# lbcb-sci/raven

Measured on NVIDIA H100. Metric: overlaps/s, higher is better.
Workload: dtype u64

## Files before the change

### profiles/index_build_split.py

```python
from __future__ import annotations

import argparse
import ctypes as C
import json
import os
import subprocess
import sys

ROOT = os.path.dirname(os.path.dirname(os.path.abspath(__file__)))
sys.path.insert(0, ROOT)

SEED = 20260924
K, W, FREQ, KMAX = 15, 5, 0.001, 32
READS, GENOME, MEAN_LEN = 200_000, 50_000_000, 10_000

KERNELS = ("TierCountKernel", "TierScatterKernel", "RadixHistogramKernel", "RadixScanBinsKernel",
           "OnesweepPass", "PartitionPass", "GroupCountKernel", "BareCountKernel",
           "IndexTableKernel", "FillLongGaps")


def card():
    try:
        out = subprocess.run(["nvidia-smi", "--query-gpu=name,power.limit,clocks.max.sm",
                              "--format=csv,noheader"], capture_output=True, text=True,
                             timeout=30).stdout.strip().splitlines()
        return out[0] if out else "unknown"
    except (OSError, subprocess.SubprocessError):
        return "unknown"


def index_sizes(eng):
    v, o, n, nk = (C.POINTER(C.c_uint64)(), C.POINTER(C.c_uint64)(), C.c_uint64(0),
                   C.c_uint64(0))
    eng._check(eng.lib.rvn_index_records(eng.h, C.byref(v), C.byref(o), C.byref(n), C.byref(nk)))
    n_a = n.value
    vmax = max(v[n_a - 1], 1) if n_a else 1
    return n_a, int(eng.stats()["index_records"]), int(vmax).bit_length()


def algorithmic_bytes(name, n, n_a, n_b, passes_a):
    if "TierCountKernel" in name:
        return 4 * n
    if "TierScatterKernel" in name:
        return 4 * n + 8 * n_a + 12 * n_a + 4 * n_b
    if "RadixHistogramKernel<unsigned int>" in name:
        return 4 * (n_a + n_b)
    if "OnesweepPass<unsigned int, unsigned long" in name:
        return passes_a * 24 * n_a
    if "OnesweepPass<unsigned int, unsigned int, false>" in name:
        return 2 * 8 * n_b
    if "PartitionPass" in name:
        return 8 * n_b
    if "GroupCountKernel" in name or "BareCountKernel" in name:
        return 4 * n_b
    if "IndexTableKernel<unsigned int, true>" in name:
        return 4 * n_a
    return None


def main():
    ap = argparse.ArgumentParser()
    ap.add_argument("--steps", type=int, default=3)
    ap.add_argument("--warmup", type=int, default=2)
    ap.add_argument("--bare-count", default="0,1,8,16")
    ap.add_argument("--out", default=None, metavar="DIR",
                    help="also write the tables as DIR/index_build_split.json")
    a = ap.parse_args()

    import torch
    from torch.profiler import ProfilerActivity, profile

    if not torch.cuda.is_available():
        raise SystemExit("index_build_split.py needs a CUDA device")
    from bench import synth
    from raven_b200 import engine

    rs = synth.make_reads(SEED, GENOME, READS, MEAN_LEN)
    stream = torch.cuda.current_stream()
    eng = engine.Engine(device=0, stream=stream.cuda_stream)
    eng.configure(K, W)
    eng.upload(rs)

    def step():
        eng.find_overlaps_and_create_piles(FREQ, KMAX, False, 0, fetch=False)

    dev = card()
    print(f"card: {dev}")
    report = {"card": dev, "settings": {}}
    for setting in a.bare_count.split(","):
        if setting != "default":
            eng.set_option("bare_count", int(setting))
        for _ in range(a.warmup):
            step()
        torch.cuda.synchronize()
        eng.set_option("reset_stats", 1)
        with profile(activities=[ProfilerActivity.CUDA]) as prof:
            for _ in range(a.steps):
                step()
            torch.cuda.synchronize()
        phases = eng.timings()
        free, total = torch.cuda.mem_get_info()
        n_a, n, bits_a = index_sizes(eng)
        n_b = n - n_a
        passes_a = -(-bits_a // 10)
        per = {}
        for e in prof.events():
            if e.device_type != torch.autograd.DeviceType.CUDA:
                continue
            if not any(k in e.name for k in KERNELS):
                continue
            d = per.setdefault(e.name, [0.0, 0])
            d[0] += (e.time_range.end - e.time_range.start) / 1e3
            d[1] += 1
        rows = []
        for name, (ms, cnt) in sorted(per.items(), key=lambda x: -x[1][0]):
            ms_step, launches = ms / a.steps, cnt / a.steps
            b = algorithmic_bytes(name, n, n_a, n_b, passes_a)
            rate = (b / (ms_step * 1e-3) / 1e12) if b and ms_step > 0 else None
            short = name.replace("(anonymous namespace)::", "").replace("void ", "")
            short = short.replace("unsigned ", "u").replace("rvn::", "").split("(")[0]
            rows.append({"kernel": short, "ms_per_step": round(ms_step, 3),
                         "launches_per_step": launches,
                         "gbytes": None if b is None else round(b / 1e9, 3),
                         "tb_per_s": None if rate is None else round(rate, 3)})
        print(f"\nbare_count={setting}: {a.steps} steps, n={n} n_a={n_a} n_b={n_b} "
              f"(tier A: {bits_a} bits, {passes_a} passes); device memory in use after the "
              f"steps {(total - free) / 2**30:.2f} GiB")
        print(f"  phases (last step, ms): index_sort {phases.get('index_sort', 0):.2f}  "
              f"index_table {phases.get('index_table', 0):.2f}")
        print(f"  {'kernel':<58} {'ms/step':>8} {'launch':>6} {'GB':>7} {'TB/s':>6}")
        for r in rows:
            print(f"  {r['kernel'][:58]:<58} {r['ms_per_step']:8.3f} {r['launches_per_step']:6.1f} "
                  f"{'' if r['gbytes'] is None else r['gbytes']:>7} "
                  f"{'' if r['tb_per_s'] is None else r['tb_per_s']:>6}")
        report["settings"][setting] = {
            "n": n, "n_a": n_a, "n_b": n_b, "phases_ms": phases, "kernels": rows,
            "device_mem_used_gib": round((total - free) / 2**30, 3)}
    if a.out:
        os.makedirs(a.out, exist_ok=True)
        with open(os.path.join(a.out, "index_build_split.json"), "w") as f:
            json.dump(report, f, indent=1)
    eng.close()


if __name__ == "__main__":
    main()
```

### raven_b200/csrc/engine.cuh

```cuda
#pragma once

#include <string>
#include <vector>

#include "../../include/raven_b200.h"
#include "common.cuh"

namespace rvn {

struct Params {
  uint32_t k = 15, w = 5, bandwidth = 500, chain = 4, matches = 100;
  uint32_t gap = 10000;
};

constexpr uint32_t kSketchTile = 2048;
constexpr uint32_t kSketchThreads = 256;
constexpr uint32_t kMaxWindow = 256;

struct PhaseTimer {
  std::vector<const char*> names;
  std::vector<float> ms;
  std::vector<std::pair<cudaEvent_t, cudaEvent_t>> pending;
  std::vector<cudaEvent_t> pool;
};

struct Ctx {
  int device = 0;
  int sms = 132;
  cudaStream_t stream = nullptr;
  bool own_stream = false;
  int64_t async_upload = 0;
  cudaStream_t copy_stream = nullptr;
  cudaEvent_t up_fence = nullptr;
  std::vector<cudaEvent_t> up_events;
  std::vector<uint32_t> up_read_end;
  uint32_t up_chunks = 0;
  bool up_pending = false;
  bool p_off_uploaded = false;
  std::string err;
  Params prm;
  bool keep_hits = false;
  rvn_stats stats{};

  uint32_t n_reads = 0;
  uint64_t n_words = 0;
  DevBuf<uint64_t> d_words, d_woff;
  DevBuf<uint32_t> d_len, d_ids;
  std::vector<uint64_t> h_woff;
  std::vector<uint32_t> h_len, h_ids;
  bool ids_identity = true;
  uint32_t res_first = 0, res_last = 0;
  std::vector<uint64_t> h_tile_off;
  DevBuf<uint64_t> d_tile_off;
  DevBuf<uint32_t> d_tile_read;
  uint32_t tiles_k = 0;

  bool s_valid = false;
  uint32_t s_first = 0, s_last = 0;
  uint64_t s_n = 0;
  DevBuf<uint64_t> s_val, s_org, s_off;
  bool s_is32 = false;
  std::vector<uint64_t> h_s_off;
  DevBuf<uint32_t> tile_cnt;
  DevBuf<uint64_t> tile_out, tile_status;

  bool q_valid = false;
  uint32_t q_first = 0, q_last = 0;
  uint64_t q_n = 0;
  DevBuf<uint64_t> q_val, q_org, q_off;
  bool q_is32 = false;
  std::vector<uint64_t> h_q_off;
  bool qt_valid = false;
  uint32_t qt_first = 0, qt_last = 0;
  DevBuf<uint64_t> qt_val;
  DevBuf<uint32_t> qt_pos;
  int t_b_low = 0;
  uint64_t group_count_min = 0;
  bool i_from_sketch = false;
  int64_t self_join = 1;
  int64_t bare_count = 1;

  bool i_valid = false;
  uint32_t i_first = 0, i_last = 0;
  uint64_t i_n = 0, i_keys = 0;
  DevBuf<uint64_t> i_val, i_org, i_val_alt, i_org_alt;
  bool i_is32 = false;
  int i_shift = 0;
  uint64_t i_limit = ~0ULL;
  DevBuf<uint32_t> t_cnt;
  DevBuf<uint64_t> t_off, t_aval, t_aorg, t_b0, t_b1, t_b2, t_narrow;
  const uint32_t* t_sorted_b = nullptr;
  uint64_t t_nb = 0;
  bool t_b_sorted = true;
  DevBuf<uint32_t> t_bstart;
  int bare_cluster = 0;
  int bare_clusters = 0;
  uint64_t tier_min_records = 1ULL << 18;
  DevBuf<uint32_t> i_bucket;
  int i_bucket_bits = 0;
  DevBuf<uint64_t> i_gaps;
  DevBuf<uint64_t> i_hist;
  uint32_t occurrence = 0xFFFFFFFFu;
  bool i_sorted_ids = false;
  bool ids_ascending = true;
  DevBuf<uint8_t> sort_tmp;

  DevBuf<uint32_t> m_cnt, m_first;
  DevBuf<uint8_t> m_filt;
  DevBuf<uint64_t> m_hit_off;
  DevBuf<uint64_t> m_sq_key, m_sq_key2;
  DevBuf<uint32_t> m_sq_idx, m_sq_idx2;
  DevBuf<uint64_t> h_grp, h_pos;
  DevBuf<uint64_t> m_read_hit_off;
  uint64_t i_gen = 0, j_gen = 0;
  uint32_t j_occurrence = 0, j_first = 0;
  std::vector<uint64_t> h_j_off;
  DevBuf<uint64_t> j_off, j_packed;
  DevBuf<uint32_t> j_cursor;
  DevBuf<uint64_t> m_scratch64;
  DevBuf<uint32_t> m_scratch32, m_fallback;
  DevBuf<uint32_t> m_desc, m_desc_cnt, m_desc_idx, m_desc_cnt2, m_desc_idx2, m_gdiag,
      m_oidx, m_oidx2;
  DevBuf<uint64_t> m_gpos, m_group_loc, m_okey, m_okey2, m_starts;
  DevBuf<uint32_t> m_bounds;
  DevBuf<rvn_overlap> m_ovl_raw, m_ovl, m_ovl_tmp;
  DevBuf<uint64_t> m_ovl_loc;
  DevBuf<uint64_t> m_ovl_off;
  DevBuf<uint64_t> m_counter;
  DevBuf<uint32_t> m_filtered;
  DevBuf<uint64_t> m_filt_off;
  DevBuf<uint64_t> scan_tmp;
  uint64_t m_hits = 0;
  uint32_t m_first_read = 0, m_last_read = 0;

  PinBuf<rvn_overlap> r_ovl;
  PinBuf<uint64_t> r_ovl_off;
  PinBuf<uint32_t> r_filtered;
  PinBuf<uint64_t> r_filt_off;
  uint64_t r_n_ovl = 0;
  bool r_valid = false;
  PinBuf<uint64_t> r_hit_grp, r_hit_pos, r_hit_off;
  uint64_t r_n_hits = 0;

  PinBuf<uint64_t> x_val, x_org, x_off;

  DevBuf<int32_t> p_diff;
  DevBuf<uint16_t> p_data;
  DevBuf<uint64_t> p_off;
  DevBuf<rvn_overlap> p_ovl;

  int g_cur = 0;
  uint64_t g_total = 0;
  DevBuf<rvn_overlap> g_list[2], g_stage;
  DevBuf<uint64_t> g_off, g_off_alt, g_rhs_off, g_t_off, g_pairs;
  DevBuf<uint32_t> g_cnt, g_kept, g_key, g_idx, g_key2, g_idx2, g_rhs_cnt,
      g_total_cnt;

  DevBuf<uint32_t> po_win_first, po_seq_begin, po_seq_end, po_cons_len, po_cov, po_list;
  DevBuf<uint64_t> po_seq_off, po_d_cons_off;
  DevBuf<uint8_t> po_bases, po_quals, po_cons, po_status, po_scratch;
  std::vector<uint64_t> po_cons_off, po_out_off;
  std::vector<uint8_t> po_h_status, po_h_cons, po_out_cons;
  std::vector<uint32_t> po_h_clen, po_h_cov, po_out_cov;
  uint64_t po_cells = 0;
  uint32_t po_n_windows = 0;
  bool po_has_cov = false, poa_valid = false;

  PinBuf<rvn_overlap> st_ovl;
  PinBuf<uint64_t> st_ovl_off;
  PinBuf<uint16_t> st_pile;
  std::vector<uint64_t> st_pile_off;
  uint64_t st_mapped = 0;
  bool st_valid = false;
  bool st_piles_on_device = false;

  uint32_t own_mod = 1, own_rem = 0;

  DevBuf<uint64_t> ds_split_val, ds_split_org, ds_qsplit_val, ds_qsplit_org;
  DevBuf<uint64_t> ds_grouped_grp, ds_grouped_pos, ds_rel_off, ds_seg_start, ds_seg_base,
      ds_bounds, ds_q_off;
  DevBuf<uint32_t> ds_masked, ds_hit_lhs, ds_read_cnt, ds_flag, ds_own_ids;
  DevBuf<rvn_overlap> ds_ovl_split, ds_merged;
  PinBuf<rvn_overlap> ds_r_ovl;
  PinBuf<uint64_t> ds_r_ovl_off, ds_r_pile_off;
  PinBuf<uint16_t> ds_r_pile;
  uint32_t ds_n_own = 0;
  bool ds_results_valid = false;
  void* x_arena = nullptr;
  uint64_t x_cap = 0;
  uint32_t x_rank = 0;
  std::vector<void*> x_peers;
  std::vector<cudaStream_t> x_streams;

  PinBuf<uint64_t> pin64;

  PhaseTimer timer;
  uint64_t launches = 0;
};

void ExclusiveScanU32(Ctx& c, const uint32_t* in, uint64_t* out, uint64_t n);
uint64_t ReadU64(Ctx& c, const uint64_t* dptr);

void TimerBegin(Ctx& c, const char* name);
void TimerEnd(Ctx& c);
void TimerCollect(Ctx& c);
void TimerReset(Ctx& c);

void EnsureTiles(Ctx& c);
void EnsureSketch(Ctx& c, uint32_t first, uint32_t last);
void WaitUpload(Ctx& c);
void EnsureMicromizers(Ctx& c, uint32_t first, uint32_t last);
void EnsureThresholds(Ctx& c, uint32_t first, uint32_t last);

void BuildIndex(Ctx& c, uint32_t first, uint32_t last, bool minhash,
                uint64_t value_limit = ~0ULL);
uint64_t MaxMicromizerValue(Ctx& c, uint32_t first, uint32_t last);
void BuildIndexFrom(Ctx& c, ValView src_val, const uint64_t* src_org, uint64_t n,
                    uint64_t index_bases, uint64_t value_limit = ~0ULL, bool count_bare = false);

int RadixSortPairs(Ctx& c, const uint32_t* src_keys, uint32_t* keys_a, uint32_t* keys_b,
                   const uint64_t* src_vals, uint64_t* vals_a, uint64_t* vals_b, uint64_t n,
                   int begin_bit, int end_bit, bool descending = false);
int RadixSortPairs(Ctx& c, const uint64_t* src_keys, uint64_t* keys_a, uint64_t* keys_b,
                   const uint64_t* src_vals, uint64_t* vals_a, uint64_t* vals_b, uint64_t n,
                   int begin_bit, int end_bit, bool descending = false);
int RadixSortPairs(Ctx& c, const uint32_t* src_keys, uint32_t* keys_a, uint32_t* keys_b,
                   const uint32_t* src_vals, uint32_t* vals_a, uint32_t* vals_b, uint64_t n,
                   int begin_bit, int end_bit, bool descending = false);
int RadixSortPairs(Ctx& c, const uint64_t* src_keys, uint64_t* keys_a, uint64_t* keys_b,
                   const uint32_t* src_vals, uint32_t* vals_a, uint32_t* vals_b, uint64_t n,
                   int begin_bit, int end_bit, bool descending = false);
int RadixSortKeys(Ctx& c, const uint32_t* src_keys, uint32_t* keys_a, uint32_t* keys_b,
                  uint64_t n, int begin_bit, int end_bit);
void RadixPartitionKeys(Ctx& c, const uint32_t* src, uint32_t* dst, uint64_t n, int begin_bit,
                        int end_bit, uint32_t* bin_start);
uint64_t* IndexHistogram(Ctx& c);
uint32_t ThresholdFromHistogram(Ctx& c, const uint64_t* h_hist, uint64_t n_keys,
                                double frequency, bool* needs_long_runs);
uint32_t FilterIndex(Ctx& c, double frequency);

void MapRange(Ctx& c, uint32_t first, uint32_t last, bool avoid_equal,
              bool avoid_symmetric, bool minhash, bool want_filtered,
              bool fetch = true);

uint64_t ChainGroupedHits(Ctx& c, const uint64_t* hg, const uint64_t* hp,
                          const uint64_t* read_hit_off,
                          const std::vector<uint64_t>& h_rho, const uint32_t* lhs_ids,
                          uint32_t nr, uint64_t n_hits, uint64_t n_q);

void GatherReset(Ctx& c);
void GatherFlush(Ctx& c, const rvn_overlap* ovl, const uint64_t* q_ovl_off,
                 uint64_t m, uint32_t k0, uint32_t k1, uint64_t kmax);
void GatherFetch(Ctx& c);

void DistSketchSplit(Ctx& c, uint32_t first, uint32_t last, int which, uint32_t parts,
                     const uint64_t** d_val, const uint64_t** d_org, uint64_t* counts);
void DistHitsSplit(Ctx& c, const uint64_t* d_qval, const uint64_t* d_qorg, uint64_t n_q,
                   bool avoid_equal, bool avoid_symmetric, uint32_t parts, uint32_t n_query,
                   const uint64_t** d_grp, const uint64_t** d_pos, const uint32_t** d_lhs,
                   uint64_t* counts);
void DistChainOwned(Ctx& c, const uint64_t* d_grp, const uint64_t* d_pos,
                    const uint32_t* d_lhs, uint64_t n_hits, uint32_t n_seg,
                    const uint64_t* h_seg_off, uint32_t mod, uint32_t rem, uint32_t n_query,
                    const rvn_overlap** d_ovl, uint64_t* n_ovl);
void DistOverlapsSplit(Ctx& c, uint32_t parts, uint32_t self, const rvn_overlap** d_out,
                       uint64_t* counts);
void DistStage1Begin(Ctx& c, uint32_t parts, uint32_t rank);
void DistStage1Add(Ctx& c, const rvn_overlap* d_ovl, uint64_t n_ovl, uint32_t n_seg,
                   const uint64_t* h_seg_off, uint32_t n_query, uint64_t kmax, uint64_t qb);
void DistStage1End(Ctx& c);
void ArenaClosePeers(Ctx& c);
void ArenaExport(Ctx& c, uint64_t bytes, void* handle64);
void ArenaImport(Ctx& c, uint32_t parts, uint32_t rank, const void* handles);
void ArenaPut(Ctx& c, uint32_t dest, uint64_t dst_off, const void* d_src, uint64_t bytes);
void ArenaFlush(Ctx& c);
void ArenaRelease(Ctx& c);

void StagePileRegions(Ctx& c, uint32_t coverage, uint32_t* h_begin, uint32_t* h_end,
                      uint16_t* h_median, uint8_t* h_invalid);
void AlignBreakingPoints(Ctx& c, uint64_t n, const uint32_t* q_read, const uint32_t* q_begin,
                         const uint32_t* q_len, const uint8_t* strand, const uint32_t* t_read,
                         const uint32_t* t_begin, const uint32_t* t_len, uint32_t window,
                         const uint64_t* bp_off, int32_t* distance, uint32_t* bp);
void EditDistanceBatch(Ctx& c, uint64_t n, const uint32_t* lhs_read, const uint32_t* lhs_begin,
                       const uint32_t* lhs_len, const uint32_t* rhs_read,
                       const uint32_t* rhs_begin, const uint32_t* rhs_len,
                       const uint8_t* strand, const int32_t* limit, int32_t* out);

void PileAddLayersDevice(Ctx& c, uint16_t* d_data, const uint64_t* d_off,
                         const uint64_t* h_off, uint32_t n_piles,
                         const rvn_overlap* d_ovl, uint64_t n_ovl);

void PoaBatch(Ctx& c, uint32_t n_windows, const uint32_t* h_win_first,
              const uint64_t* h_seq_off, const uint8_t* h_bases, const uint8_t* h_quals,
              const uint32_t* h_seq_begin, const uint32_t* h_seq_end, int m, int n,
              int gap, bool trim, bool tgs, bool want_coverage);

void KmerComplexity(Ctx& c, const uint32_t* h_read_idx, const uint32_t* h_pos,
                    uint64_t n, uint32_t k, uint8_t* h_keep);

}
```

### raven_b200/csrc/index.cu

```cuda
#include <algorithm>
#include <cmath>

#include <cooperative_groups.h>

#include "engine.cuh"

namespace rvn {

namespace {

constexpr int kThreads = 256;

constexpr uint32_t kHistBins = 1u << 16;
constexpr uint32_t kSmemBins = 1024;

constexpr uint32_t kShortGap = 1024;
constexpr uint32_t kMaxLongGaps = 1u << 20;

template <typename ValT, bool kFill>
__global__ void __launch_bounds__(kThreads)
IndexTableKernel(const ValT* __restrict__ val, uint64_t n, int shift,
                 uint32_t n_buckets, uint32_t* __restrict__ bucket,
                 unsigned long long* __restrict__ hist, uint64_t* __restrict__ gaps) {
  __shared__ uint32_t sh[kSmemBins];
  __shared__ uint32_t keys;
  __shared__ uint32_t warp_first[kThreads / 32];
  for (uint32_t i = threadIdx.x; i < kSmemBins; i += kThreads) sh[i] = 0;
  if (threadIdx.x == 0) keys = 0;
  __syncthreads();
  const uint64_t stride = static_cast<uint64_t>(gridDim.x) * kThreads;
  for (uint64_t base = static_cast<uint64_t>(blockIdx.x) * kThreads; base <= n; base += stride) {
  const uint64_t i = base + threadIdx.x;
  bool start = false;
  uint32_t len = 0;
  uint64_t fill_lo = 0, mine = 0;
  uint32_t fill_cnt = 0;
  if (i <= n) {
    const uint64_t prev = i == 0 ? 0 : val[i - 1];
    const uint64_t cur = i == n ? 0 : val[i];
    const uint64_t lo = i == 0 ? 0 : (prev >> shift) + 1;
    const uint64_t hi = i == n ? n_buckets : (cur >> shift);
    if (kFill && hi >= lo) {
      if (hi + 1 - lo <= kShortGap) {
        fill_lo = lo;
        fill_cnt = static_cast<uint32_t>(hi + 1 - lo);
      } else {
        const unsigned long long g = atomicAdd(&hist[kHistBins + 1], 1ULL);
        if (g < kMaxLongGaps) {
          gaps[3 * g] = lo;
          gaps[3 * g + 1] = hi;
          gaps[3 * g + 2] = i;
        } else {
          for (uint64_t b = lo; b <= hi; ++b) bucket[b] = static_cast<uint32_t>(i);
        }
      }
    }
    start = i < n && (i == 0 || cur != prev);
    mine = cur;
  }
  {
    const uint32_t lane = threadIdx.x & 31, wid = threadIdx.x >> 5;
    const uint32_t marks = __ballot_sync(0xFFFFFFFFu, start || i == n);
    if (lane == 0) warp_first[wid] = marks ? static_cast<uint32_t>(__ffs(marks) - 1) : 32u;
    __syncthreads();
    if (start) {
      const uint32_t above = lane == 31 ? 0u : (marks & ~((2u << lane) - 1u));
      if (above) {
        len = static_cast<uint32_t>(__ffs(above) - 1) - lane;
      } else {
        len = 32 - lane;
        uint32_t w2 = wid + 1;
        while (w2 < kThreads / 32 && warp_first[w2] == 32u) {
          len += 32;
          ++w2;
        }
        if (w2 < kThreads / 32) {
          len += warp_first[w2];
        } else {
          uint64_t pos = base + kThreads;
          while (len < kHistBins - 1 && pos < n && val[pos] == mine) {
            ++pos;
            ++len;
          }
        }
      }
      if (len > kHistBins - 1) len = kHistBins - 1;
    }
    __syncthreads();
  }
  {
    const uint32_t lane = threadIdx.x & 31;
    uint32_t incl = fill_cnt;
#pragma unroll
    for (int d = 1; d < 32; d <<= 1) {
      const uint32_t o = __shfl_up_sync(0xFFFFFFFFu, incl, d);
      if (lane >= static_cast<uint32_t>(d)) incl += o;
    }
    const uint32_t rel = incl - fill_cnt;
    const uint32_t total = __shfl_sync(0xFFFFFFFFu, incl, 31);
    for (uint32_t t0 = 0; t0 < total; t0 += 32) {
      const uint32_t t = t0 + lane;
      uint32_t q = 0;
#pragma unroll
      for (uint32_t step = 16; step > 0; step >>= 1) {
        const uint32_t r = __shfl_sync(0xFFFFFFFFu, rel, q + step);
        if (r <= t) q += step;
      }
      const uint32_t qrel = __shfl_sync(0xFFFFFFFFu, rel, q);
      const uint64_t qlo = __shfl_sync(0xFFFFFFFFu, fill_lo, q);
      if (kFill && t < total) bucket[qlo + (t - qrel)] = static_cast<uint32_t>(base + (threadIdx.x & ~31u) + q);
    }
  }
  const uint32_t starts = __ballot_sync(0xFFFFFFFFu, start);
  if (start) {
    const uint32_t same = __match_any_sync(starts, len);
    if ((threadIdx.x & 31) == static_cast<uint32_t>(__ffs(same) - 1)) {
      if (len < kSmemBins) {
        atomicAdd(&sh[len], static_cast<uint32_t>(__popc(same)));
      } else {
        atomicAdd(&hist[len], static_cast<unsigned long long>(__popc(same)));
      }
    }
  }
  if ((threadIdx.x & 31) == 0 && starts) atomicAdd(&keys, static_cast<uint32_t>(__popc(starts)));

  }
  __syncthreads();
  for (uint32_t b = threadIdx.x; b < kSmemBins; b += kThreads) {
    if (sh[b]) atomicAdd(&hist[b], static_cast<unsigned long long>(sh[b]));
  }
  if (threadIdx.x == 0 && keys) atomicAdd(&hist[kHistBins], static_cast<unsigned long long>(keys));
}

__global__ void __launch_bounds__(kThreads)
FillLongGaps(const uint64_t* __restrict__ gaps, uint32_t* __restrict__ bucket) {
  const uint64_t lo = gaps[3ULL * blockIdx.x], hi = gaps[3ULL * blockIdx.x + 1];
  const uint32_t v = static_cast<uint32_t>(gaps[3ULL * blockIdx.x + 2]);
  for (uint64_t b = lo + threadIdx.x; b <= hi; b += kThreads) bucket[b] = v;
}

template <typename ValT>
__global__ void CollectLongRuns(const ValT* __restrict__ val, uint64_t n,
                                unsigned long long* __restrict__ counter,
                                uint32_t* __restrict__ out) {
  const uint64_t i = static_cast<uint64_t>(blockIdx.x) * blockDim.x + threadIdx.x;
  if (i >= n || (i > 0 && val[i] == val[i - 1])) return;
  if (i + (kHistBins - 2) >= n || val[i + (kHistBins - 2)] != val[i]) return;
  uint64_t len = kHistBins - 1;
  while (i + len < n && val[i + len] == val[i]) ++len;
  out[atomicAdd(counter, 1ULL)] = static_cast<uint32_t>(len);
}

__global__ void NarrowValuesKernel(const uint64_t* __restrict__ in, uint64_t n,
                                   uint32_t* __restrict__ out) {
  const uint64_t i = static_cast<uint64_t>(blockIdx.x) * blockDim.x + threadIdx.x;
  if (i < n) out[i] = static_cast<uint32_t>(in[i]);
}

constexpr uint32_t kTierTile = 4096;

__global__ void __launch_bounds__(kThreads)
TierCountKernel(const uint32_t* __restrict__ val, uint64_t n, uint32_t limit,
                uint32_t* __restrict__ tile_cnt) {
  __shared__ uint32_t sm[34];
  const uint64_t base = static_cast<uint64_t>(blockIdx.x) * kTierTile;
  uint32_t mine = 0;
#pragma unroll
  for (uint32_t i = 0; i < kTierTile / kThreads; ++i) {
    const uint64_t idx = base + i * kThreads + threadIdx.x;
    mine += (idx < n && val[idx] <= limit) ? 1u : 0u;
  }
  uint32_t total;
  BlockExclusiveSum<uint32_t, kThreads>(mine, sm, &total);
  if (threadIdx.x == 0) tile_cnt[blockIdx.x] = total;
}

__global__ void __launch_bounds__(kThreads, 4)
TierScatterKernel(const uint32_t* __restrict__ val, const uint64_t* __restrict__ org, uint64_t n,
                  uint32_t limit, const uint64_t* __restrict__ tile_off_a,
                  uint32_t* __restrict__ a_val, uint64_t* __restrict__ a_org,
                  uint32_t* __restrict__ b_val) {
  __shared__ uint32_t warp_a[kThreads / 32];
  const uint32_t lane = threadIdx.x & 31, warp = threadIdx.x >> 5;
  constexpr uint32_t kWarpSpan = kTierTile / (kThreads / 32);
  const uint64_t tile_base = static_cast<uint64_t>(blockIdx.x) * kTierTile;
  const uint64_t warp_base = tile_base + warp * kWarpSpan;
  uint32_t v[kWarpSpan / 32];
  uint32_t cnt = 0;
#pragma unroll
  for (uint32_t i = 0; i < kWarpSpan / 32; ++i) {
    const uint64_t idx = warp_base + i * 32 + lane;
    v[i] = idx < n ? val[idx] : 0xFFFFFFFFu;
  }
#pragma unroll
  for (uint32_t i = 0; i < kWarpSpan / 32; ++i) {
    const uint64_t idx = warp_base + i * 32 + lane;
    cnt += __popc(__ballot_sync(0xFFFFFFFFu, idx < n && v[i] <= limit));
  }
  if (lane == 0) warp_a[warp] = cnt;
  __syncthreads();
  uint64_t a_at = tile_off_a[blockIdx.x];
  for (uint32_t w = 0; w < warp; ++w) a_at += warp_a[w];
  uint64_t b_at = warp_base - a_at;
#pragma unroll
  for (uint32_t h = 0; h < kWarpSpan / 32; h += 8) {
    uint64_t o[8];
#pragma unroll
    for (uint32_t u = 0; u < 8; ++u) {
      const uint64_t idx = warp_base + (h + u) * 32 + lane;
      o[u] = (idx < n && v[h + u] <= limit) ? org[idx] : 0;
    }
#pragma unroll
    for (uint32_t u = 0; u < 8; ++u) {
      const uint32_t i = h + u;
      const uint64_t idx = warp_base + i * 32 + lane;
      const bool in = idx < n;
      const bool is_a = in && v[i] <= limit;
      const uint32_t ma = __ballot_sync(0xFFFFFFFFu, is_a);
      const uint32_t mb = __ballot_sync(0xFFFFFFFFu, in && !is_a);
      const uint32_t below = (1u << lane) - 1u;
      if (is_a) {
        const uint64_t d = a_at + __popc(ma & below);
        a_val[d] = v[i];
        a_org[d] = o[u];
      } else if (in) {
        b_val[b_at + __popc(mb & below)] = v[i];
      }
      a_at += __popc(ma);
      b_at += __popc(mb);
    }
  }
}

__global__ void MaxU64Kernel(const uint64_t* __restrict__ v, uint64_t n,
                             unsigned long long* __restrict__ out) {
  unsigned long long m = 0;
  const uint64_t stride = static_cast<uint64_t>(gridDim.x) * blockDim.x;
  for (uint64_t i = static_cast<uint64_t>(blockIdx.x) * blockDim.x + threadIdx.x; i < n;
       i += stride) {
    m = max(m, static_cast<unsigned long long>(v[i]));
  }
#pragma unroll
  for (int d = 16; d > 0; d >>= 1) m = max(m, __shfl_xor_sync(0xFFFFFFFFu, m, d));
  if ((threadIdx.x & 31) == 0) atomicMax(out, m);
}

constexpr uint32_t kGroupChunk = 4096;
constexpr int kGroupLowBits = 10;

__global__ void __launch_bounds__(kThreads)
GroupCountKernel(const uint32_t* __restrict__ key, uint64_t n, unsigned long long* __restrict__ hist) {
  __shared__ uint32_t sh[kSmemBins];
  __shared__ __align__(16) uint32_t cnt[kThreads / 32][1u << kGroupLowBits];
  __shared__ uint32_t keys_total;
  for (uint32_t i = threadIdx.x; i < kSmemBins; i += kThreads) sh[i] = 0;
  if (threadIdx.x == 0) keys_total = 0;
  __syncthreads();
  const uint32_t lane = threadIdx.x & 31, wid = threadIdx.x >> 5;
  uint32_t* my = cnt[wid];
  const uint32_t low_mask = (1u << kGroupLowBits) - 1;
  uint32_t h1 = 0, h2 = 0, h3 = 0, h4 = 0, nkeys = 0;
  const uint64_t n_chunks = (n + kGroupChunk - 1) / kGroupChunk;
  for (uint64_t chunk = static_cast<uint64_t>(blockIdx.x) * (kThreads / 32) + wid; chunk < n_chunks;
       chunk += static_cast<uint64_t>(gridDim.x) * (kThreads / 32)) {
    const uint64_t start = chunk * kGroupChunk;
    const uint64_t end = min(n, start + kGroupChunk);
    uint64_t pos = start;
    if (start > 0) {
      const uint32_t gprev = key[start - 1] >> kGroupLowBits;
      while (true) {
        const uint64_t idx = pos + lane;
        const bool in = idx < n && (key[idx] >> kGroupLowBits) == gprev;
        const uint32_t m = __ballot_sync(0xFFFFFFFFu, in);
        const uint32_t c = m == 0xFFFFFFFFu ? 32u : static_cast<uint32_t>(__ffs(~m) - 1);
        pos += c;
        if (c < 32) break;
      }
    }
    while (pos < end) {
      const uint32_t g = key[pos] >> kGroupLowBits;
      uint4* my4 = reinterpret_cast<uint4*>(my);
#pragma unroll
      for (uint32_t t = 0; t < (1u << kGroupLowBits) / 128; ++t) my4[t * 32 + lane] = make_uint4(0, 0, 0, 0);
      __syncwarp();
      bool open = true;
      while (open) {
        uint32_t k4[4];
#pragma unroll
        for (uint32_t u = 0; u < 4; ++u) {
          const uint64_t idx = pos + u * 32 + lane;
          k4[u] = idx < n ? key[idx] : ~(g << kGroupLowBits);
        }
#pragma unroll
        for (uint32_t u = 0; u < 4; ++u) {
          if (open) {
            const bool in = (k4[u] >> kGroupLowBits) == g;
            const uint32_t m = __ballot_sync(0xFFFFFFFFu, in);
            if (in) atomicAdd(&my[k4[u] & low_mask], 1u);
            const uint32_t c = m == 0xFFFFFFFFu ? 32u : static_cast<uint32_t>(__ffs(~m) - 1);
            pos += c;
            open = c == 32;
          }
        }
      }
      __syncwarp();
#pragma unroll
      for (uint32_t t = 0; t < (1u << kGroupLowBits) / 128; ++t) {
        const uint4 q = my4[t * 32 + lane];
        if ((q.x | q.y | q.z | q.w) == 0) continue;
        const uint32_t cs[4] = {q.x, q.y, q.z, q.w};
#pragma unroll
        for (int x = 0; x < 4; ++x) {
          const uint32_t c = cs[x];
          if (c == 0) continue;
          ++nkeys;
          if (c <= 4) {
            h1 += c == 1;
            h2 += c == 2;
            h3 += c == 3;
            h4 += c == 4;
          } else if (c < kSmemBins) {
            atomicAdd(&sh[c], 1u);
          } else {
            atomicAdd(&hist[min(c, kHistBins - 1)], 1ULL);
          }
        }
      }
      __syncwarp();
    }
  }
#pragma unroll
  for (int d = 16; d > 0; d >>= 1) {
    h1 += __shfl_xor_sync(0xFFFFFFFFu, h1, d);
    h2 += __shfl_xor_sync(0xFFFFFFFFu, h2, d);
    h3 += __shfl_xor_sync(0xFFFFFFFFu, h3, d);
    h4 += __shfl_xor_sync(0xFFFFFFFFu, h4, d);
    nkeys += __shfl_xor_sync(0xFFFFFFFFu, nkeys, d);
  }
  if (lane == 0) {
    atomicAdd(&sh[1], h1);
    atomicAdd(&sh[2], h2);
    atomicAdd(&sh[3], h3);
    atomicAdd(&sh[4], h4);
    atomicAdd(&keys_total, nkeys);
  }
  __syncthreads();
  for (uint32_t i = threadIdx.x; i < kSmemBins; i += kThreads) {
    if (sh[i]) atomicAdd(&hist[i], static_cast<unsigned long long>(sh[i]));
  }
  if (threadIdx.x == 0 && keys_total) {
    atomicAdd(&hist[kHistBins], static_cast<unsigned long long>(keys_total));
  }
}

constexpr int kBareBucketBits = 10;
constexpr int kBareThreads = 1024;
constexpr int kBareSlotBits = 15;

__global__ void __launch_bounds__(kBareThreads, 1)
BareCountKernel(const uint32_t* __restrict__ key, uint64_t n, const uint32_t* __restrict__ bstart,
                uint32_t first_bucket, uint32_t n_buckets, int span_bits, int slot_bits,
                unsigned long long* __restrict__ hist) {
  extern __shared__ __align__(16) uint32_t bare_smem[];
  __shared__ uint32_t keys_total;
  namespace cg = cooperative_groups;
  cg::cluster_group cluster = cg::this_cluster();
  const uint32_t csize = cluster.num_blocks();
  const uint32_t crank = cluster.block_rank();
  const uint32_t n_slots = 1u << slot_bits;
  uint32_t* ctr = bare_smem;
  uint32_t* sh = bare_smem + n_slots;
  for (uint32_t i = threadIdx.x; i < n_slots; i += kBareThreads) ctr[i] = 0;
  for (uint32_t i = threadIdx.x; i < kSmemBins; i += kBareThreads) sh[i] = 0;
  if (threadIdx.x == 0) keys_total = 0;
  const uint32_t ctr_addr = static_cast<uint32_t>(__cvta_generic_to_shared(ctr));
  const uint32_t span_mask = (1u << span_bits) - 1u;
  const uint32_t sweep_span = n_slots * csize;
  const uint32_t slot_mask = n_slots - 1u;
  uint32_t h1 = 0, h2 = 0, h3 = 0, h4 = 0, nkeys = 0;
  cluster.sync();
  const uint32_t n_clusters = gridDim.x / csize;
  for (uint32_t b = first_bucket + blockIdx.x / csize; b < n_buckets; b += n_clusters) {
    const uint64_t lo = bstart ? bstart[b] : 0;
    const uint64_t hi = bstart && b + 1 < n_buckets ? bstart[b + 1] : n;
    if (lo >= hi) continue;
    for (uint64_t s0 = 0; s0 <= span_mask; s0 += sweep_span) {
      constexpr int kUnroll = 4;
      const uint64_t stride = static_cast<uint64_t>(csize) * kBareThreads;
      for (uint64_t i0 = lo + crank * kBareThreads + threadIdx.x; i0 < hi; i0 += kUnroll * stride) {
        uint32_t k4[kUnroll];
#pragma unroll
        for (int u = 0; u < kUnroll; ++u) {
          const uint64_t i = i0 + u * stride;
          k4[u] = i < hi ? key[i] : 0u;
        }
#pragma unroll
        for (int u = 0; u < kUnroll; ++u) {
          const uint64_t v = static_cast<uint64_t>(k4[u] & span_mask) - s0;
          if (i0 + u * stride < hi && v < sweep_span) {
            const uint32_t owner = static_cast<uint32_t>(v) >> slot_bits;
            const uint32_t local = ctr_addr + 4u * (static_cast<uint32_t>(v) & slot_mask);
            uint32_t remote;
            asm volatile("mapa.shared::cluster.u32 %0, %1, %2;" : "=r"(remote) : "r"(local), "r"(owner));
            asm volatile("red.relaxed.cluster.shared::cluster.add.u32 [%0], 1;" ::"r"(remote) : "memory");
          }
        }
      }
      cluster.sync();
      for (uint32_t t = threadIdx.x; t < n_slots; t += kBareThreads) {
        const uint32_t c = ctr[t];
        if (c == 0) continue;
        ctr[t] = 0;
        ++nkeys;
        if (c <= 4) {
          h1 += c == 1;
          h2 += c == 2;
          h3 += c == 3;
          h4 += c == 4;
        } else if (c < kSmemBins) {
          atomicAdd(&sh[c], 1u);
        } else {
          atomicAdd(&hist[min(c, kHistBins - 1)], 1ULL);
        }
      }
      cluster.sync();
    }
  }
#pragma unroll
  for (int d = 16; d > 0; d >>= 1) {
    h1 += __shfl_xor_sync(0xFFFFFFFFu, h1, d);
    h2 += __shfl_xor_sync(0xFFFFFFFFu, h2, d);
    h3 += __shfl_xor_sync(0xFFFFFFFFu, h3, d);
    h4 += __shfl_xor_sync(0xFFFFFFFFu, h4, d);
    nkeys += __shfl_xor_sync(0xFFFFFFFFu, nkeys, d);
  }
  if ((threadIdx.x & 31) == 0) {
    atomicAdd(&sh[1], h1);
    atomicAdd(&sh[2], h2);
    atomicAdd(&sh[3], h3);
    atomicAdd(&sh[4], h4);
    atomicAdd(&keys_total, nkeys);
  }
  __syncthreads();
  for (uint32_t i = threadIdx.x; i < kSmemBins; i += kBareThreads) {
    if (sh[i]) atomicAdd(&hist[i], static_cast<unsigned long long>(sh[i]));
  }
  if (threadIdx.x == 0 && keys_total) {
    atomicAdd(&hist[kHistBins], static_cast<unsigned long long>(keys_total));
  }
}

void BareCount(Ctx& c, const uint32_t* keys, uint64_t n, int key_bits, uint32_t limit,
               const uint32_t* bstart, unsigned long long* hist) {
  const int span_bits = bstart ? key_bits - kBareBucketBits : key_bits;
  const uint32_t n_buckets = bstart ? (1u << kBareBucketBits) : 1u;
  const uint32_t first_bucket = bstart ? (limit >> span_bits) : 0u;
  if (c.bare_cluster == 0) {
    const int size = c.bare_count > 1 ? static_cast<int>(c.bare_count) : 8;
    const size_t smem = ((1u << kBareSlotBits) + kSmemBins) * sizeof(uint32_t);
    RVN_CUDA(cudaFuncSetAttribute(BareCountKernel, cudaFuncAttributeMaxDynamicSharedMemorySize,
                                  static_cast<int>(smem)));
    RVN_CUDA(cudaFuncSetAttribute(BareCountKernel, cudaFuncAttributeNonPortableClusterSizeAllowed, 1));
    cudaLaunchConfig_t cfg = {};
    cfg.gridDim = dim3(static_cast<unsigned>(size));
    cfg.blockDim = dim3(kBareThreads);
    cfg.dynamicSmemBytes = smem;
    cudaLaunchAttribute attr[1];
    attr[0].id = cudaLaunchAttributeClusterDimension;
    attr[0].val.clusterDim.x = static_cast<unsigned>(size);
    attr[0].val.clusterDim.y = 1;
    attr[0].val.clusterDim.z = 1;
    cfg.attrs = attr;
    cfg.numAttrs = 1;
    int clusters = 0;
    RVN_CUDA(cudaOccupancyMaxActiveClusters(&clusters, BareCountKernel, &cfg));
    if (clusters < 1) throw CudaError("BareCountKernel: a cluster does not fit the device");
    c.bare_cluster = size;
    c.bare_clusters = clusters;
  }
  const int csize = c.bare_cluster;
  int log_c = 0;
  while ((1 << log_c) < csize) ++log_c;
  const int slot_bits = std::max(0, std::min(kBareSlotBits, span_bits - log_c));
  const unsigned clusters =
      static_cast<unsigned>(std::min<uint64_t>(n_buckets - first_bucket, c.bare_clusters));
  cudaLaunchConfig_t cfg = {};
  cfg.gridDim = dim3(clusters * csize);
  cfg.blockDim = dim3(kBareThreads);
  cfg.dynamicSmemBytes = ((1u << slot_bits) + kSmemBins) * sizeof(uint32_t);
  cfg.stream = c.stream;
  cudaLaunchAttribute attr[1];
  attr[0].id = cudaLaunchAttributeClusterDimension;
  attr[0].val.clusterDim.x = static_cast<unsigned>(csize);
  attr[0].val.clusterDim.y = 1;
  attr[0].val.clusterDim.z = 1;
  cfg.attrs = attr;
  cfg.numAttrs = 1;
  RVN_CUDA(cudaLaunchKernelEx(&cfg, BareCountKernel, keys, n, bstart, first_bucket, n_buckets,
                              span_bits, slot_bits, hist));
  RVN_LAUNCH_CHECK();
  ++c.launches;
}

}

uint64_t MaxMicromizerValue(Ctx& c, uint32_t first, uint32_t last) {
  EnsureThresholds(c, first, last);
  if (last <= first) return 0;
  if (!c.s_is32) return ~0ULL;
  uint64_t* w = c.m_counter.reserve(8);
  RVN_CUDA(cudaMemsetAsync(w, 0, sizeof(uint64_t), c.stream));
  const uint64_t n = last - first;
  MaxU64Kernel<<<std::min<unsigned>(CeilDiv(n, 256), c.sms * 8), 256, 0, c.stream>>>(
      c.qt_val.get(), n, reinterpret_cast<unsigned long long*>(w));
  RVN_LAUNCH_CHECK();
  ++c.launches;
  return ReadU64(c, w);
}

void BuildIndex(Ctx& c, uint32_t first, uint32_t last, bool minhash, uint64_t value_limit) {
  c.i_valid = false;
  c.occurrence = 0xFFFFFFFFu;
  EnsureSketch(c, first, last);
  ValView src_val{c.s_val.get(), c.s_is32 ? 1 : 0};
  const uint64_t* src_org = c.s_org.get();
  uint64_t n = c.s_n;
  if (minhash) {
    EnsureMicromizers(c, first, last);
    src_val = ValView{c.q_val.get(), c.q_is32 ? 1 : 0};
    src_org = c.q_org.get();
    n = c.q_n;
  }
  uint64_t bases = 0;
  for (uint32_t r = first; r < last; ++r) bases += c.h_len[r];
  c.i_first = first;
  c.i_last = last;
  BuildIndexFrom(c, src_val, src_org, n, bases, minhash ? ~0ULL : value_limit,
                 true);
  c.i_sorted_ids = c.ids_ascending;
  c.i_from_sketch = !minhash;
}

void BuildIndexFrom(Ctx& c, ValView src_val, const uint64_t* src_org, uint64_t n,
                    uint64_t index_bases, uint64_t value_limit, bool count_bare) {
  c.i_valid = false;
  c.i_sorted_ids = false;
  c.i_from_sketch = false;
  c.occurrence = 0xFFFFFFFFu;
  ++c.i_gen;
  if (n >= 0xFFFFFFFFULL) {
    throw LimitError("index batch holds 2^32 or more minimizers");
  }
  c.i_n = n;
  c.i_keys = 0;
  if (!src_val.is32 && 2 * c.prm.k <= 30 && n > 0) {
    uint32_t* narrow = reinterpret_cast<uint32_t*>(c.t_narrow.reserve(n / 2 + 2));
    NarrowValuesKernel<<<CeilDiv(n, kThreads), kThreads, 0, c.stream>>>(
        static_cast<const uint64_t*>(src_val.p), n, narrow);
    RVN_LAUNCH_CHECK();
    ++c.launches;
    src_val = ValView{narrow, 1};
  }
  const bool is32 = src_val.is32 != 0;
  c.i_is32 = is32;

  const int key_bits = static_cast<int>(2 * c.prm.k);
  const uint64_t value_mask = key_bits >= 64 ? ~0ULL : ((1ULL << key_bits) - 1);
  const bool tiered = is32 && value_limit < value_mask && n >= c.tier_min_records;
  const uint32_t limit32 = static_cast<uint32_t>(value_limit);
  c.i_limit = tiered ? value_limit : ~0ULL;
  uint64_t n_a = n, n_b = 0;
  const uint32_t* sorted_b = nullptr;
  const bool bare = tiered && count_bare && c.bare_count != 0;
  const uint32_t* bstart = nullptr;

  TimerBegin(c, "index_sort");
  if (tiered) {
    const uint32_t* src32 = static_cast<const uint32_t*>(src_val.p);
    const uint64_t tiles = (n + kTierTile - 1) / kTierTile;
    uint32_t* tcnt = c.t_cnt.reserve(tiles + 1);
    uint64_t* toff = c.t_off.reserve(tiles + 2);
    TierCountKernel<<<static_cast<unsigned>(tiles), kThreads, 0, c.stream>>>(src32, n, limit32,
                                                                          tcnt);
    ExclusiveScanU32(c, tcnt, toff, tiles);
    n_a = ReadU64(c, toff + tiles);
    n_b = n - n_a;
    uint32_t* a_val = reinterpret_cast<uint32_t*>(c.t_aval.reserve(n_a / 2 + 2));
    uint64_t* a_org = c.t_aorg.reserve(n_a + 1);
    uint32_t* b_src = reinterpret_cast<uint32_t*>(c.t_b0.reserve(n_b / 2 + 2));
    TierScatterKernel<<<static_cast<unsigned>(tiles), kThreads, 0, c.stream>>>(
        src32, src_org, n, limit32, toff, a_val, a_org, b_src);
    RVN_LAUNCH_CHECK();
    c.launches += 2;
    int bits_a = 1;
    while (bits_a < key_bits && (value_limit >> bits_a) != 0) ++bits_a;
    c.i_val.reserve(n_a / 2 + 2);
    c.i_val_alt.reserve(n_a / 2 + 2);
    c.i_org.reserve(n_a + 1);
    c.i_org_alt.reserve(n_a + 1);
    if (n_a > 0) {
      const int where = RadixSortPairs(c, a_val, reinterpret_cast<uint32_t*>(c.i_val.get()),
                                       reinterpret_cast<uint32_t*>(c.i_val_alt.get()), a_org,
                                       c.i_org.get(), c.i_org_alt.get(), n_a, 0, bits_a);
      if (where == 1) {
        c.i_val.swap(c.i_val_alt);
        c.i_org.swap(c.i_org_alt);
      }
    }
    uint32_t* b1 = reinterpret_cast<uint32_t*>(c.t_b1.reserve(n_b / 2 + 2));
    if (bare) {
      c.t_b2.release();
      c.t_b_low = 0;
      c.t_b_sorted = false;
      sorted_b = n_b > 0 ? b_src : nullptr;
      if (n_b > 0 && key_bits > 2 * kBareBucketBits) {
        uint32_t* starts = c.t_bstart.reserve(1u << kBareBucketBits);
        RadixPartitionKeys(c, b_src, b1, n_b, key_bits - kBareBucketBits, key_bits, starts);
        sorted_b = b1;
        bstart = starts;
      }
    } else {
      uint32_t* b2 = reinterpret_cast<uint32_t*>(c.t_b2.reserve(n_b / 2 + 2));
      const uint64_t n_groups = ((value_mask - value_limit) >> kGroupLowBits) + 1;
      c.t_b_low = (key_bits > 2 * kGroupLowBits && n_b / n_groups >= c.group_count_min)
                      ? kGroupLowBits
                      : 0;
      c.t_b_sorted = c.t_b_low == 0;
      if (n_b > 0) {
        const int where = RadixSortKeys(c, b_src, b1, b2, n_b, c.t_b_low, key_bits);
        sorted_b = where < 0 ? b_src : (where == 0 ? b1 : b2);
      }
    }
    c.t_sorted_b = sorted_b;
    c.t_nb = n_b;
  } else {
    const uint64_t val_elems = is32 ? n / 2 + 2 : n + 1;
    c.i_val.reserve(val_elems);
    c.i_val_alt.reserve(val_elems);
    c.i_org.reserve(n + 1);
    c.i_org_alt.reserve(n + 1);
    if (n > 0) {
      int where;
      if (is32) {
        where = RadixSortPairs(c, static_cast<const uint32_t*>(src_val.p),
                               reinterpret_cast<uint32_t*>(c.i_val.get()),
                               reinterpret_cast<uint32_t*>(c.i_val_alt.get()), src_org,
                               c.i_org.get(), c.i_org_alt.get(), n, 0, key_bits);
      } else {
        where = RadixSortPairs(c, static_cast<const uint64_t*>(src_val.p), c.i_val.get(),
                               c.i_val_alt.get(), src_org, c.i_org.get(), c.i_org_alt.get(), n, 0,
                               key_bits);
      }
      if (where == 1) {
        c.i_val.swap(c.i_val_alt);
        c.i_org.swap(c.i_org_alt);
      }
    }
    c.t_sorted_b = nullptr;
    c.t_nb = 0;
    c.t_b_sorted = true;
  }
  c.i_n = n_a;
  TimerEnd(c);
  const uint64_t* kv = c.i_val.get();

  TimerBegin(c, "index_table");
  int top_bits = key_bits;
  if (tiered) {
    top_bits = 1;
    while (top_bits < key_bits && (value_limit >> top_bits) != 0) ++top_bits;
  }
  int bits = 8;
  while (bits < 28 && (1ULL << (bits + 1)) <= n_a) ++bits;
  bits = std::min<int>(bits, top_bits);
  c.i_bucket_bits = bits;
  const int shift = top_bits - bits;
  c.i_shift = shift;
  const uint32_t n_buckets =
      tiered ? static_cast<uint32_t>((value_limit >> shift) + 1) : (1u << bits);
  uint32_t* bucket = c.i_bucket.reserve(n_buckets + 2ULL);
  static_assert(sizeof(unsigned long long) == sizeof(uint64_t), "");
  uint64_t* hist = c.i_hist.reserve(kHistBins + 8);
  RVN_CUDA(cudaMemsetAsync(hist, 0, (kHistBins + 8) * sizeof(uint64_t), c.stream));
  uint64_t* gaps = c.i_gaps.reserve(3ULL * kMaxLongGaps);
  const unsigned grid = std::min<unsigned>(CeilDiv(n_a + 1, kThreads), c.sms * 8);
  if (is32) {
    IndexTableKernel<uint32_t, true><<<grid, kThreads, 0, c.stream>>>(
        reinterpret_cast<const uint32_t*>(kv), n_a, shift, n_buckets, bucket,
        reinterpret_cast<unsigned long long*>(hist), gaps);
    if (tiered && n_b > 0) {
      if (bare) {
        BareCount(c, sorted_b, n_b, key_bits, limit32, bstart,
                  reinterpret_cast<unsigned long long*>(hist));
        --c.launches;
      } else if (c.t_b_low) {
        GroupCountKernel<<<std::min<unsigned>(CeilDiv(n_b, kGroupChunk * (kThreads / 32)), c.sms * 6),
                           kThreads, 0, c.stream>>>(sorted_b, n_b,
                                                    reinterpret_cast<unsigned long long*>(hist));
      } else {
        IndexTableKernel<uint32_t, false>
            <<<std::min<unsigned>(CeilDiv(n_b + 1, kThreads), c.sms * 8), kThreads, 0, c.stream>>>(
                sorted_b, n_b, 0, 0, nullptr, reinterpret_cast<unsigned long long*>(hist), nullptr);
      }
      ++c.launches;
    }
  } else {
    IndexTableKernel<uint64_t, true><<<grid, kThreads, 0, c.stream>>>(
        kv, n_a, shift, n_buckets, bucket, reinterpret_cast<unsigned long long*>(hist), gaps);
  }
  RVN_LAUNCH_CHECK();
  ++c.launches;
  uint64_t* hk = c.pin64.reserve(8);
  RVN_CUDA(cudaMemcpyAsync(hk, hist + kHistBins, 2 * sizeof(uint64_t), cudaMemcpyDeviceToHost,
                           c.stream));
  RVN_CUDA(cudaStreamSynchronize(c.stream));
  c.i_keys = hk[0];
  const uint64_t n_long = std::min<uint64_t>(hk[1], kMaxLongGaps);
  if (n_long) {
    FillLongGaps<<<static_cast<unsigned>(n_long), kThreads, 0, c.stream>>>(gaps, bucket);
    RVN_LAUNCH_CHECK();
    ++c.launches;
  }
  TimerEnd(c);

  c.stats.index_bases = index_bases;
  c.stats.index_records = n;
  c.stats.index_keys = c.i_keys;
  c.i_valid = true;
}

uint64_t* IndexHistogram(Ctx& c) {
  return c.i_hist.get();
}

uint32_t ThresholdFromHistogram(Ctx& c, const uint64_t* h, uint64_t n_keys,
                                double frequency, bool* needs_long_runs) {
  (void)c;
  *needs_long_runs = false;
  std::size_t rank = static_cast<std::size_t>((1 - frequency) * static_cast<double>(n_keys));
  if (rank >= n_keys) rank = n_keys - 1;
  uint64_t cum = 0;
  for (uint32_t len = 0; len + 1 < kHistBins; ++len) {
    cum += h[len];
    if (cum > rank) return len + 1;
  }
  *needs_long_runs = true;
  return 0;
}

uint32_t FilterIndex(Ctx& c, double frequency) {
  if (!(0 <= frequency && frequency <= 1)) {
    throw InvalidArgument(
        "[ram::MinimizerEngine::Filter] error: invalid frequency");
  }
  if (!c.i_valid) throw StateError("Filter before Minimize");
  if (frequency == 0 || c.i_keys == 0) {
    c.occurrence = 0xFFFFFFFFu;
    return c.occurrence;
  }
  uint64_t* hist = IndexHistogram(c);
  std::vector<uint64_t> h(kHistBins);
  RVN_CUDA(cudaMemcpyAsync(h.data(), hist, kHistBins * sizeof(uint64_t),
                           cudaMemcpyDeviceToHost, c.stream));
  RVN_CUDA(cudaStreamSynchronize(c.stream));
  bool long_runs = false;
  uint32_t occ = ThresholdFromHistogram(c, h.data(), c.i_keys, frequency, &long_runs);
  if (long_runs) {
    uint64_t cum = 0;
    for (uint32_t len = 0; len + 1 < kHistBins; ++len) cum += h[len];
    std::size_t rank = static_cast<std::size_t>((1 - frequency) * static_cast<double>(c.i_keys));
    if (rank >= c.i_keys) rank = c.i_keys - 1;
    const uint64_t n_long = h[kHistBins - 1];
    uint32_t* out = c.m_cnt.reserve(n_long + 1);
    uint64_t* counter = c.m_counter.reserve(8);
    RVN_CUDA(cudaMemsetAsync(counter, 0, sizeof(uint64_t), c.stream));
    if (c.i_is32) {
      CollectLongRuns<uint32_t><<<CeilDiv(c.i_n, kThreads), kThreads, 0, c.stream>>>(
          reinterpret_cast<const uint32_t*>(c.i_val.get()), c.i_n,
          reinterpret_cast<unsigned long long*>(counter), out);
      if (c.t_sorted_b && c.t_nb && !c.t_b_sorted) {
        uint32_t* bufs[3] = {reinterpret_cast<uint32_t*>(c.t_b0.get()),
                             reinterpret_cast<uint32_t*>(c.t_b1.get()),
                             reinterpret_cast<uint32_t*>(c.t_b2.get())};
        uint32_t* src = nullptr;
        for (uint32_t* p : bufs) {
          if (p == c.t_sorted_b) src = p;
        }
        uint32_t* other = src == bufs[0] ? bufs[1] : bufs[0];
        const int where = RadixSortKeys(c, src, other, src, c.t_nb, 0,
                                        static_cast<int>(2 * c.prm.k));
        c.t_sorted_b = where == 0 ? other : src;
        c.t_b_low = 0;
        c.t_b_sorted = true;
      }
      if (c.t_sorted_b && c.t_nb) {
        CollectLongRuns<uint32_t><<<CeilDiv(c.t_nb, kThreads), kThreads, 0, c.stream>>>(
            c.t_sorted_b, c.t_nb, reinterpret_cast<unsigned long long*>(counter), out);
      }
    } else {
      CollectLongRuns<uint64_t><<<CeilDiv(c.i_n, kThreads), kThreads, 0, c.stream>>>(
          c.i_val.get(), c.i_n, reinterpret_cast<unsigned long long*>(counter), out);
    }
    RVN_LAUNCH_CHECK();
    ++c.launches;
    std::vector<uint32_t> lens(n_long);
    RVN_CUDA(cudaMemcpyAsync(lens.data(), out, n_long * sizeof(uint32_t),
                             cudaMemcpyDeviceToHost, c.stream));
    RVN_CUDA(cudaStreamSynchronize(c.stream));
    std::sort(lens.begin(), lens.end());
    occ = lens[rank - cum] + 1;
  }
  c.occurrence = occ;
  c.stats.occurrence = c.occurrence;
  return c.occurrence;
}

}
```

### raven_b200/csrc/radix.cu

```cuda
#include <algorithm>

#include "engine.cuh"

namespace rvn {

namespace {

constexpr int kRadixMaxBits = 10;
constexpr int kBins = 1 << kRadixMaxBits;
constexpr int kThreads = 256;
constexpr int kWarps = kThreads / 32;
constexpr int kBinsPerThread = kBins / kThreads;
constexpr int kMaxPasses = 8;
template <typename KeyT>
struct Items {
  static constexpr int value = sizeof(KeyT) == 4 ? 32 : 16;
};

constexpr uint32_t kFlagAggregate = 1u << 30;
constexpr uint32_t kFlagPrefix = 2u << 30;
constexpr uint32_t kFlagMask = 3u << 30;
constexpr uint32_t kValueMask = ~kFlagMask;

struct PassPlan {
  int n_passes;
  int begin[kMaxPasses];
  int bits[kMaxPasses];
};

template <typename KeyT>
__device__ __forceinline__ uint32_t Digit(KeyT key, KeyT flip, int begin, uint32_t mask) {
  return static_cast<uint32_t>((key ^ flip) >> begin) & mask;
}

template <typename KeyT>
__global__ void __launch_bounds__(kThreads)
RadixHistogramKernel(const KeyT* __restrict__ keys, uint64_t n, PassPlan plan, KeyT flip,
                     unsigned long long* __restrict__ hist) {
  extern __shared__ uint32_t sh_hist[];
  const int total = plan.n_passes * kBins;
  for (int i = threadIdx.x; i < total; i += kThreads) sh_hist[i] = 0;
  __syncthreads();
  const uint64_t stride = static_cast<uint64_t>(gridDim.x) * kThreads;
  for (uint64_t i = static_cast<uint64_t>(blockIdx.x) * kThreads + threadIdx.x; i < n;
       i += stride) {
    const KeyT k = keys[i];
#pragma unroll
    for (int p = 0; p < kMaxPasses; ++p) {
      if (p < plan.n_passes) {
        atomicAdd(&sh_hist[p * kBins + Digit<KeyT>(k, flip, plan.begin[p],
                                                    (1u << plan.bits[p]) - 1u)], 1u);
      }
    }
  }
  __syncthreads();
  for (int i = threadIdx.x; i < total; i += kThreads) {
    if (sh_hist[i]) atomicAdd(&hist[i], static_cast<unsigned long long>(sh_hist[i]));
  }
}

__global__ void __launch_bounds__(kBins)
RadixScanBinsKernel(const unsigned long long* __restrict__ hist, int n_passes,
                    uint32_t* __restrict__ bin_base) {
  __shared__ uint32_t sm[34];
  for (int p = 0; p < n_passes; ++p) {
    const uint32_t v = static_cast<uint32_t>(hist[p * kBins + threadIdx.x]);
    uint32_t total;
    const uint32_t ex = BlockExclusiveSum<uint32_t, kBins>(v, sm, &total);
    bin_base[p * kBins + threadIdx.x] = ex;
  }
}

__device__ __forceinline__ void ChainTileCounts(uint32_t* __restrict__ status, uint32_t tile,
                                                const uint32_t (&cnt)[kBinsPerThread],
                                                uint32_t (&excl)[kBinsPerThread]) {
  uint4* st4 = reinterpret_cast<uint4*>(status);
  const uint64_t my4 = static_cast<uint64_t>(tile) * (kBins / 4) + threadIdx.x;
#pragma unroll
  for (int j = 0; j < kBinsPerThread; ++j) excl[j] = 0;
  static_assert(kBinsPerThread == 4, "one uint4 of status words per thread");
  if (tile > 0) {
    uint4 agg;
    agg.x = kFlagAggregate | cnt[0];
    agg.y = kFlagAggregate | cnt[1];
    agg.z = kFlagAggregate | cnt[2];
    agg.w = kFlagAggregate | cnt[3];
    asm volatile("st.volatile.global.v4.u32 [%0], {%1, %2, %3, %4};" ::"l"(st4 + my4),
                 "r"(agg.x), "r"(agg.y), "r"(agg.z), "r"(agg.w)
                 : "memory");
    constexpr int kLook = 4;
    uint32_t open = 0xF;
    int64_t p = static_cast<int64_t>(tile) - 1;
    while (open) {
      uint4 v[kLook];
#pragma unroll
      for (int u = 0; u < kLook; ++u) {
        const int64_t q = p - u;
        if (q >= 0) {
          const uint4* src = st4 + static_cast<uint64_t>(q) * (kBins / 4) + threadIdx.x;
          asm volatile("ld.volatile.global.v4.u32 {%0, %1, %2, %3}, [%4];"
                       : "=r"(v[u].x), "=r"(v[u].y), "=r"(v[u].z), "=r"(v[u].w)
                       : "l"(src)
                       : "memory");
        } else {
          v[u] = make_uint4(kFlagPrefix, kFlagPrefix, kFlagPrefix, kFlagPrefix);
        }
      }
      int used = 0;
#pragma unroll
      for (int u = 0; u < kLook; ++u) {
        const uint32_t vv[4] = {v[u].x, v[u].y, v[u].z, v[u].w};
        const bool ready = (vv[0] & kFlagMask) && (vv[1] & kFlagMask) && (vv[2] & kFlagMask) &&
                           (vv[3] & kFlagMask);
        if (used == u && ready && open) {
#pragma unroll
          for (int j = 0; j < kBinsPerThread; ++j) {
            if (open & (1u << j)) {
              excl[j] += vv[j] & kValueMask;
              if ((vv[j] & kFlagMask) == kFlagPrefix) open &= ~(1u << j);
            }
          }
          used = u + 1;
        }
      }
      p -= used;
    }
  }
  uint4 pre;
  pre.x = kFlagPrefix | (excl[0] + cnt[0]);
  pre.y = kFlagPrefix | (excl[1] + cnt[1]);
  pre.z = kFlagPrefix | (excl[2] + cnt[2]);
  pre.w = kFlagPrefix | (excl[3] + cnt[3]);
  asm volatile("st.volatile.global.v4.u32 [%0], {%1, %2, %3, %4};" ::"l"(st4 + my4), "r"(pre.x),
               "r"(pre.y), "r"(pre.z), "r"(pre.w)
               : "memory");
}

template <typename KeyT, typename ValT, bool HAS_VAL>
struct __align__(16) PassSmem {
  static constexpr int kTile = kThreads * Items<KeyT>::value;
  uint16_t warp_hist[kWarps][kBins];
  uint32_t bin_off[kBins];
  uint32_t bin_dst[kBins];
  uint32_t scan[34];
  uint32_t tile;
  uint16_t slot_digit[HAS_VAL ? kTile : 2];
  union {
    KeyT keys[kTile];
    ValT vals[HAS_VAL ? kTile : 1];
  } stage;
};

template <typename KeyT, typename ValT, bool HAS_VAL>
__global__ void __launch_bounds__(kThreads, 2)
OnesweepPass(const KeyT* __restrict__ keys_in, KeyT* __restrict__ keys_out,
             const ValT* __restrict__ vals_in, ValT* __restrict__ vals_out, uint32_t n,
             KeyT flip, int begin_bit, int pass_bits, const uint32_t* __restrict__ bin_base,
             uint32_t* __restrict__ bin_next, uint32_t* __restrict__ status,
             unsigned int* __restrict__ ticket) {
  extern __shared__ __align__(16) unsigned char smem_raw[];
  using Smem = PassSmem<KeyT, ValT, HAS_VAL>;
  constexpr int kItems = Items<KeyT>::value;
  constexpr int kTile = kThreads * kItems;
  constexpr int kWarpTile = 32 * kItems;
  Smem& sm = *reinterpret_cast<Smem*>(smem_raw);
  const uint32_t lane = threadIdx.x & 31, warp = threadIdx.x >> 5;
  const uint32_t lanemask_lt = (1u << lane) - 1u;
  const uint32_t dmask = (1u << pass_bits) - 1u;

  if (threadIdx.x == 0) sm.tile = atomicAdd(ticket, 1u);
  {
    uint32_t* w = reinterpret_cast<uint32_t*>(&sm.warp_hist[0][0]);
#pragma unroll
    for (int i = 0; i < kWarps * kBins / 2 / kThreads; ++i) w[i * kThreads + threadIdx.x] = 0;
  }
  __syncthreads();
  const uint32_t tile = sm.tile;
  const uint64_t tile_base = static_cast<uint64_t>(tile) * kTile;
  const uint32_t tile_count =
      static_cast<uint32_t>(min(static_cast<uint64_t>(kTile), static_cast<uint64_t>(n) - tile_base));

  KeyT key[kItems];
  const uint32_t warp_base = warp * kWarpTile;
#pragma unroll
  for (int i = 0; i < kItems; ++i) {
    const uint32_t t = warp_base + i * 32 + lane;
    key[i] = t < tile_count ? keys_in[tile_base + t] : static_cast<KeyT>(0);
  }

  constexpr int kHalf = kItems / 2;
  ValT early[HAS_VAL ? kHalf : 1];
  if (HAS_VAL) {
#pragma unroll
    for (int i = 0; i < kHalf; ++i) {
      const uint32_t t = warp_base + i * 32 + lane;
      early[i] = t < tile_count ? vals_in[tile_base + t] : ValT(0);
    }
  }

  uint16_t rank[kItems];
  uint16_t* my_hist = sm.warp_hist[warp];
#pragma unroll
  for (int i = 0; i < kItems; ++i) {
    const uint32_t t = warp_base + i * 32 + lane;
    const bool valid = t < tile_count;
    const uint32_t d = valid ? Digit<KeyT>(key[i], flip, begin_bit, dmask) : 0u;
    uint32_t peers = __ballot_sync(0xFFFFFFFFu, valid);
#pragma unroll
    for (int bit = 0; bit < kRadixMaxBits; ++bit) {
      const bool one = (d >> bit) & 1u;
      const uint32_t vote = __ballot_sync(0xFFFFFFFFu, one);
      peers &= one ? vote : ~vote;
    }
    if (!valid) peers = 1u << lane;
    const uint32_t leader = __ffs(peers) - 1;
    uint32_t before = 0;
    if (lane == leader && valid) {
      before = my_hist[d];
      my_hist[d] = static_cast<uint16_t>(before + __popc(peers));
    }
    before = __shfl_sync(0xFFFFFFFFu, before, leader);
    rank[i] = static_cast<uint16_t>(before + __popc(peers & lanemask_lt));
    __syncwarp();
  }
  __syncthreads();

  uint32_t cnt[kBinsPerThread];
  uint32_t mine = 0;
#pragma unroll
  for (int j = 0; j < kBinsPerThread; ++j) {
    const uint32_t b = threadIdx.x * kBinsPerThread + j;
    uint32_t c = 0;
#pragma unroll
    for (int w = 0; w < kWarps; ++w) {
      const uint32_t x = sm.warp_hist[w][b];
      sm.warp_hist[w][b] = static_cast<uint16_t>(c);
      c += x;
    }
    cnt[j] = c;
    mine += c;
  }
  uint32_t total;
  uint32_t ex = BlockExclusiveSum<uint32_t, kThreads>(mine, sm.scan, &total);
#pragma unroll
  for (int j = 0; j < kBinsPerThread; ++j) {
    sm.bin_off[threadIdx.x * kBinsPerThread + j] = ex;
    ex += cnt[j];
  }

  {
    uint32_t excl[kBinsPerThread];
    ChainTileCounts(status, tile, cnt, excl);
#pragma unroll
    for (int j = 0; j < kBinsPerThread; ++j) {
      const uint32_t b = threadIdx.x * kBinsPerThread + j;
      const uint32_t base = bin_base[b];
      sm.bin_dst[b] = base + excl[j] - sm.bin_off[b];
      if (tile == gridDim.x - 1) bin_next[b] = base + excl[j] + cnt[j];
    }
  }
  __syncthreads();

#pragma unroll
  for (int i = 0; i < kItems; ++i) {
    const uint32_t t = warp_base + i * 32 + lane;
    if (t < tile_count) {
      const uint32_t d = Digit<KeyT>(key[i], flip, begin_bit, dmask);
      const uint32_t slot = sm.bin_off[d] + sm.warp_hist[warp][d] + rank[i];
      rank[i] = static_cast<uint16_t>(slot);
      if (HAS_VAL) sm.slot_digit[slot] = static_cast<uint16_t>(d);
    }
  }

  if (HAS_VAL) {
    ValT late[kHalf];
#pragma unroll
    for (int i = 0; i < kHalf; ++i) {
      const uint32_t t = warp_base + (kHalf + i) * 32 + lane;
      late[i] = t < tile_count ? vals_in[tile_base + t] : ValT(0);
    }
#pragma unroll
    for (int i = 0; i < kHalf; ++i) {
      const uint32_t t = warp_base + i * 32 + lane;
      if (t < tile_count) sm.stage.vals[rank[i]] = early[i];
    }
#pragma unroll
    for (int i = 0; i < kHalf; ++i) {
      const uint32_t t = warp_base + (kHalf + i) * 32 + lane;
      if (t < tile_count) sm.stage.vals[rank[kHalf + i]] = late[i];
    }
    __syncthreads();
#pragma unroll
    for (int i = 0; i < kItems; ++i) {
      const uint32_t s = i * kThreads + threadIdx.x;
      if (s < tile_count) vals_out[sm.bin_dst[sm.slot_digit[s]] + s] = sm.stage.vals[s];
    }
    __syncthreads();
  }

#pragma unroll
  for (int i = 0; i < kItems; ++i) {
    const uint32_t t = warp_base + i * 32 + lane;
    if (t < tile_count) sm.stage.keys[rank[i]] = key[i];
  }
  __syncthreads();
#pragma unroll
  for (int i = 0; i < kItems; ++i) {
    const uint32_t s = i * kThreads + threadIdx.x;
    if (s < tile_count) {
      const KeyT k = sm.stage.keys[s];
      keys_out[sm.bin_dst[Digit<KeyT>(k, flip, begin_bit, dmask)] + s] = k;
    }
  }
}

struct PartitionSmem {
  uint32_t bin_cnt[kBins];
  uint32_t bin_off[kBins];
  uint32_t bin_dst[kBins];
  uint32_t scan[34];
  uint32_t tile;
  uint32_t keys[kThreads * Items<uint32_t>::value];
};

__global__ void __launch_bounds__(kThreads, 2)
PartitionPass(const uint32_t* __restrict__ keys_in, uint32_t* __restrict__ keys_out, uint32_t n,
              int begin_bit, int pass_bits, const uint32_t* __restrict__ bin_base,
              uint32_t* __restrict__ bin_next, uint32_t* __restrict__ status,
              unsigned int* __restrict__ ticket) {
  extern __shared__ __align__(16) unsigned char smem_raw[];
  PartitionSmem& sm = *reinterpret_cast<PartitionSmem*>(smem_raw);
  constexpr int kItems = Items<uint32_t>::value;
  constexpr int kTile = kThreads * kItems;
  constexpr int kWarpTile = 32 * kItems;
  const uint32_t lane = threadIdx.x & 31, warp = threadIdx.x >> 5;
  const uint32_t dmask = (1u << pass_bits) - 1u;

  if (threadIdx.x == 0) sm.tile = atomicAdd(ticket, 1u);
#pragma unroll
  for (int j = 0; j < kBinsPerThread; ++j) sm.bin_cnt[j * kThreads + threadIdx.x] = 0;
  __syncthreads();
  const uint32_t tile = sm.tile;
  const uint64_t tile_base = static_cast<uint64_t>(tile) * kTile;
  const uint32_t tile_count =
      static_cast<uint32_t>(min(static_cast<uint64_t>(kTile), static_cast<uint64_t>(n) - tile_base));

  uint32_t key[kItems];
  const uint32_t warp_base = warp * kWarpTile;
#pragma unroll
  for (int i = 0; i < kItems; ++i) {
    const uint32_t t = warp_base + i * 32 + lane;
    key[i] = t < tile_count ? keys_in[tile_base + t] : 0u;
  }
  uint16_t rank[kItems];
#pragma unroll
  for (int i = 0; i < kItems; ++i) {
    const uint32_t t = warp_base + i * 32 + lane;
    if (t < tile_count) {
      rank[i] = static_cast<uint16_t>(atomicAdd(&sm.bin_cnt[(key[i] >> begin_bit) & dmask], 1u));
    }
  }
  __syncthreads();

  uint32_t cnt[kBinsPerThread];
  uint32_t mine = 0;
#pragma unroll
  for (int j = 0; j < kBinsPerThread; ++j) {
    cnt[j] = sm.bin_cnt[threadIdx.x * kBinsPerThread + j];
    mine += cnt[j];
  }
  uint32_t total;
  uint32_t ex = BlockExclusiveSum<uint32_t, kThreads>(mine, sm.scan, &total);
#pragma unroll
  for (int j = 0; j < kBinsPerThread; ++j) {
    sm.bin_off[threadIdx.x * kBinsPerThread + j] = ex;
    ex += cnt[j];
  }
  {
    uint32_t excl[kBinsPerThread];
    ChainTileCounts(status, tile, cnt, excl);
#pragma unroll
    for (int j = 0; j < kBinsPerThread; ++j) {
      const uint32_t b = threadIdx.x * kBinsPerThread + j;
      const uint32_t base = bin_base[b];
      sm.bin_dst[b] = base + excl[j] - sm.bin_off[b];
      if (tile == gridDim.x - 1) bin_next[b] = base + excl[j] + cnt[j];
    }
  }
  __syncthreads();

#pragma unroll
  for (int i = 0; i < kItems; ++i) {
    const uint32_t t = warp_base + i * 32 + lane;
    if (t < tile_count) sm.keys[sm.bin_off[(key[i] >> begin_bit) & dmask] + rank[i]] = key[i];
  }
  __syncthreads();
#pragma unroll
  for (int i = 0; i < kItems; ++i) {
    const uint32_t s = i * kThreads + threadIdx.x;
    if (s < tile_count) {
      const uint32_t k = sm.keys[s];
      keys_out[sm.bin_dst[(k >> begin_bit) & dmask] + s] = k;
    }
  }
}

PassPlan MakePlan(int begin_bit, int end_bit) {
  PassPlan plan{};
  const int total = std::max(0, end_bit - begin_bit);
  const int np = (total + kRadixMaxBits - 1) / kRadixMaxBits;
  if (np > kMaxPasses) throw InvalidArgument("radix sort: too many key bits");
  plan.n_passes = np;
  int at = begin_bit;
  for (int p = 0; p < np; ++p) {
    const int b = (total - (at - begin_bit) + (np - p) - 1) / (np - p);
    plan.begin[p] = at;
    plan.bits[p] = b;
    at += b;
  }
  return plan;
}

template <typename KeyT, typename ValT, bool HAS_VAL>
int SortImpl(Ctx& c, const KeyT* src_keys, KeyT* keys_a, KeyT* keys_b, const ValT* src_vals,
             ValT* vals_a, ValT* vals_b, uint64_t n, int begin_bit, int end_bit,
             bool descending) {
  if (n >= 0xFFFFFFFFULL) throw LimitError("radix sort of 2^32 or more records");
  const PassPlan plan = MakePlan(begin_bit, end_bit);
  if (plan.n_passes == 0 || n == 0) return -1;
  using Smem = PassSmem<KeyT, ValT, HAS_VAL>;
  constexpr uint64_t kTile = Smem::kTile;
  const KeyT flip = descending ? static_cast<KeyT>(~static_cast<KeyT>(0)) : static_cast<KeyT>(0);
  const uint64_t portion = ((1ULL << 30) - 1) / kTile * kTile;
  const uint64_t n_portions = (n + portion - 1) / portion;
  const uint64_t max_tiles = (std::min(n, portion) + kTile - 1) / kTile;
  const size_t hist_bytes = sizeof(uint64_t) * plan.n_passes * kBins;
  const size_t base_bytes = sizeof(uint32_t) * plan.n_passes * kBins;
  const size_t ticket_bytes = sizeof(unsigned int) * kMaxPasses * 8;
  if (plan.n_passes * n_portions > kMaxPasses * 8) throw LimitError("radix sort: too many launches");
  const size_t status_bytes = sizeof(uint32_t) * max_tiles * kBins;
  const size_t head = hist_bytes + 2 * base_bytes + ticket_bytes;
  uint8_t* scratch = c.sort_tmp.reserve(head + status_bytes + 256);
  auto* hist = reinterpret_cast<unsigned long long*>(scratch);
  uint32_t* bases[2] = {reinterpret_cast<uint32_t*>(scratch + hist_bytes),
                        reinterpret_cast<uint32_t*>(scratch + hist_bytes + base_bytes)};
  auto* ticket = reinterpret_cast<unsigned int*>(scratch + hist_bytes + 2 * base_bytes);
  auto* status = reinterpret_cast<uint32_t*>(scratch + head);
  RVN_CUDA(cudaMemsetAsync(scratch, 0, head, c.stream));
  const unsigned hgrid =
      static_cast<unsigned>(std::min<uint64_t>((n + kThreads - 1) / kThreads, c.sms * 8));
  RadixHistogramKernel<KeyT><<<hgrid, kThreads, sizeof(uint32_t) * plan.n_passes * kBins,
                               c.stream>>>(src_keys, n, plan, flip, hist);
  RadixScanBinsKernel<<<1, kBins, 0, c.stream>>>(hist, plan.n_passes, bases[0]);
  RVN_LAUNCH_CHECK();
  c.launches += 2;

  auto kern = OnesweepPass<KeyT, ValT, HAS_VAL>;
  RVN_CUDA(cudaFuncSetAttribute(kern, cudaFuncAttributeMaxDynamicSharedMemorySize,
                                static_cast<int>(sizeof(Smem))));
  const KeyT* kin = src_keys;
  const ValT* vin = src_vals;
  int where = -1;
  unsigned launch = 0;
  for (int p = 0; p < plan.n_passes; ++p) {
    const int to = where == 0 ? 1 : 0;
    KeyT* kout = to == 0 ? keys_a : keys_b;
    ValT* vout = to == 0 ? vals_a : vals_b;
    int cur = 0;
    for (uint64_t q = 0; q < n_portions; ++q) {
      const uint64_t first = q * portion;
      const uint64_t cnt = std::min(portion, n - first);
      const uint64_t tiles = (cnt + kTile - 1) / kTile;
      RVN_CUDA(cudaMemsetAsync(status, 0, sizeof(uint32_t) * tiles * kBins, c.stream));
      kern<<<static_cast<unsigned>(tiles), kThreads, sizeof(Smem), c.stream>>>(
          kin + first, kout, HAS_VAL ? vin + first : vin, vout, static_cast<uint32_t>(cnt), flip,
          plan.begin[p], plan.bits[p], bases[cur] + p * kBins, bases[cur ^ 1] + p * kBins, status,
          ticket + launch);
      RVN_LAUNCH_CHECK();
      ++c.launches;
      ++launch;
      cur ^= 1;
    }
    kin = kout;
    vin = vout;
    where = to;
  }
  return where;
}

}

int RadixSortPairs(Ctx& c, const uint32_t* src_keys, uint32_t* keys_a, uint32_t* keys_b,
                   const uint64_t* src_vals, uint64_t* vals_a, uint64_t* vals_b, uint64_t n,
                   int begin_bit, int end_bit, bool descending) {
  return SortImpl<uint32_t, uint64_t, true>(c, src_keys, keys_a, keys_b, src_vals, vals_a, vals_b,
                                            n, begin_bit, end_bit, descending);
}
int RadixSortPairs(Ctx& c, const uint64_t* src_keys, uint64_t* keys_a, uint64_t* keys_b,
                   const uint64_t* src_vals, uint64_t* vals_a, uint64_t* vals_b, uint64_t n,
                   int begin_bit, int end_bit, bool descending) {
  return SortImpl<uint64_t, uint64_t, true>(c, src_keys, keys_a, keys_b, src_vals, vals_a, vals_b,
                                            n, begin_bit, end_bit, descending);
}
int RadixSortPairs(Ctx& c, const uint32_t* src_keys, uint32_t* keys_a, uint32_t* keys_b,
                   const uint32_t* src_vals, uint32_t* vals_a, uint32_t* vals_b, uint64_t n,
                   int begin_bit, int end_bit, bool descending) {
  return SortImpl<uint32_t, uint32_t, true>(c, src_keys, keys_a, keys_b, src_vals, vals_a, vals_b,
                                            n, begin_bit, end_bit, descending);
}
int RadixSortPairs(Ctx& c, const uint64_t* src_keys, uint64_t* keys_a, uint64_t* keys_b,
                   const uint32_t* src_vals, uint32_t* vals_a, uint32_t* vals_b, uint64_t n,
                   int begin_bit, int end_bit, bool descending) {
  return SortImpl<uint64_t, uint32_t, true>(c, src_keys, keys_a, keys_b, src_vals, vals_a, vals_b,
                                            n, begin_bit, end_bit, descending);
}
int RadixSortKeys(Ctx& c, const uint32_t* src_keys, uint32_t* keys_a, uint32_t* keys_b, uint64_t n,
                  int begin_bit, int end_bit) {
  return SortImpl<uint32_t, uint32_t, false>(c, src_keys, keys_a, keys_b, nullptr, nullptr, nullptr,
                                             n, begin_bit, end_bit, false);
}

void RadixPartitionKeys(Ctx& c, const uint32_t* src, uint32_t* dst, uint64_t n, int begin_bit,
                        int end_bit, uint32_t* bin_start) {
  if (n >= 0xFFFFFFFFULL) throw LimitError("radix partition of 2^32 or more records");
  if (end_bit - begin_bit < 1 || end_bit - begin_bit > kRadixMaxBits) {
    throw InvalidArgument("radix partition: 1 to 10 key bits");
  }
  PassPlan plan{};
  plan.n_passes = 1;
  plan.begin[0] = begin_bit;
  plan.bits[0] = end_bit - begin_bit;
  constexpr uint64_t kTile = kThreads * Items<uint32_t>::value;
  const uint64_t portion = ((1ULL << 30) - 1) / kTile * kTile;
  const uint64_t n_portions = (n + portion - 1) / portion;
  const uint64_t max_tiles = (std::min(n, portion) + kTile - 1) / kTile;
  const size_t hist_bytes = sizeof(uint64_t) * kBins;
  const size_t base_bytes = sizeof(uint32_t) * kBins;
  const size_t ticket_bytes = sizeof(unsigned int) * kMaxPasses * 8;
  if (n_portions > kMaxPasses * 8) throw LimitError("radix partition: too many launches");
  const size_t head = hist_bytes + 2 * base_bytes + ticket_bytes;
  const size_t status_bytes = sizeof(uint32_t) * max_tiles * kBins;
  uint8_t* scratch = c.sort_tmp.reserve(head + status_bytes + 256);
  auto* hist = reinterpret_cast<unsigned long long*>(scratch);
  uint32_t* bases[2] = {reinterpret_cast<uint32_t*>(scratch + hist_bytes),
                        reinterpret_cast<uint32_t*>(scratch + hist_bytes + base_bytes)};
  auto* ticket = reinterpret_cast<unsigned int*>(scratch + hist_bytes + 2 * base_bytes);
  auto* status = reinterpret_cast<uint32_t*>(scratch + head);
  RVN_CUDA(cudaMemsetAsync(scratch, 0, head, c.stream));
  if (n == 0) {
    RVN_CUDA(cudaMemsetAsync(bin_start, 0, base_bytes, c.stream));
    return;
  }
  const unsigned hgrid =
      static_cast<unsigned>(std::min<uint64_t>((n + kThreads - 1) / kThreads, c.sms * 8));
  RadixHistogramKernel<uint32_t><<<hgrid, kThreads, sizeof(uint32_t) * kBins, c.stream>>>(
      src, n, plan, 0u, hist);
  RadixScanBinsKernel<<<1, kBins, 0, c.stream>>>(hist, 1, bases[0]);
  RVN_LAUNCH_CHECK();
  c.launches += 2;
  RVN_CUDA(cudaMemcpyAsync(bin_start, bases[0], base_bytes, cudaMemcpyDeviceToDevice, c.stream));
  RVN_CUDA(cudaFuncSetAttribute(PartitionPass, cudaFuncAttributeMaxDynamicSharedMemorySize,
                                static_cast<int>(sizeof(PartitionSmem))));
  int cur = 0;
  for (uint64_t q = 0; q < n_portions; ++q) {
    const uint64_t first = q * portion;
    const uint64_t cnt = std::min(portion, n - first);
    const uint64_t tiles = (cnt + kTile - 1) / kTile;
    RVN_CUDA(cudaMemsetAsync(status, 0, sizeof(uint32_t) * tiles * kBins, c.stream));
    PartitionPass<<<static_cast<unsigned>(tiles), kThreads, sizeof(PartitionSmem), c.stream>>>(
        src + first, dst, static_cast<uint32_t>(cnt), plan.begin[0], plan.bits[0], bases[cur],
        bases[cur ^ 1], status, ticket + q);
    RVN_LAUNCH_CHECK();
    ++c.launches;
    cur ^= 1;
  }
}

}
```

Measured before the change: 56.09 million.

## Fuse tier split into radix sort first pass and shared histogram

Drops the separate tier count/scatter kernels that copied keys below and above the frequency limit into intermediate buffers. A single histogram kernel now counts the split and builds the digit histograms for both tiers at once. The first onesweep/partition pass of each tier then reads the original key array and filters records by the limit as it scatters. This saves a full read/write of the index arrays and a separate histogram pass, at the cost of more complex filtered first passes and a host sync to read the tier counts.

Result: no change. 56.16 million, median of 6 (+0.1%).

```diff
diff --git a/profiles/index_build_split.py b/profiles/index_build_split.py
--- a/profiles/index_build_split.py
+++ b/profiles/index_build_split.py
@@ -14,9 +14,9 @@
 K, W, FREQ, KMAX = 15, 5, 0.001, 32
 READS, GENOME, MEAN_LEN = 200_000, 50_000_000, 10_000
 
-KERNELS = ("TierCountKernel", "TierScatterKernel", "RadixHistogramKernel", "RadixScanBinsKernel",
-           "OnesweepPass", "PartitionPass", "GroupCountKernel", "BareCountKernel",
-           "IndexTableKernel", "FillLongGaps")
+KERNELS = ("TierCountKernel", "TierScatterKernel", "SplitHistogramKernel", "RadixHistogramKernel",
+           "RadixScanBinsKernel", "OnesweepPass", "PartitionPass", "GroupCountKernel",
+           "BareCountKernel", "IndexTableKernel", "FillLongGaps")
 
 
 def card():
@@ -38,17 +38,25 @@
     return n_a, int(eng.stats()["index_records"]), int(vmax).bit_length()
 
 
-def algorithmic_bytes(name, n, n_a, n_b, passes_a):
+def algorithmic_bytes(name, n, n_a, n_b, passes_a, split):
     if "TierCountKernel" in name:
         return 4 * n
     if "TierScatterKernel" in name:
         return 4 * n + 8 * n_a + 12 * n_a + 4 * n_b
+    if "SplitHistogramKernel" in name:
+        return 4 * n
     if "RadixHistogramKernel<unsigned int>" in name:
-        return 4 * (n_a + n_b)
+        return None if split else 4 * (n_a + n_b)
+    if "OnesweepPass<unsigned int, unsigned long, true, 1>" in name:
+        return 4 * n + 8 * n_a + 12 * n_a
     if "OnesweepPass<unsigned int, unsigned long" in name:
-        return passes_a * 24 * n_a
-    if "OnesweepPass<unsigned int, unsigned int, false>" in name:
-        return 2 * 8 * n_b
+        return (passes_a - (1 if split else 0)) * 24 * n_a
+    if "OnesweepPass<unsigned int, unsigned int, false, 2>" in name:
+        return 4 * n + 4 * n_b
+    if "OnesweepPass<unsigned int, unsigned int, false" in name:
+        return (1 if split else 2) * 8 * n_b
+    if "PartitionPass<true>" in name:
+        return 4 * n + 4 * n_b
     if "PartitionPass" in name:
         return 8 * n_b
     if "GroupCountKernel" in name or "BareCountKernel" in name:
@@ -66,6 +74,9 @@
     ap.add_argument("--out", default=None, metavar="DIR",
                     help="also write the tables as DIR/index_build_split.json")
     a = ap.parse_args()
+
+    import threading
+    import time
 
     import torch
     from torch.profiler import ProfilerActivity, profile
@@ -94,17 +105,32 @@
             step()
         torch.cuda.synchronize()
         eng.set_option("reset_stats", 1)
+        peak = [0]
+        done = threading.Event()
+
+        def poll():
+            while not done.is_set():
+                f, t = torch.cuda.mem_get_info()
+                peak[0] = max(peak[0], t - f)
+                time.sleep(0.001)
+
+        poller = threading.Thread(target=poll)
+        poller.start()
         with profile(activities=[ProfilerActivity.CUDA]) as prof:
             for _ in range(a.steps):
                 step()
             torch.cuda.synchronize()
+        done.set()
+        poller.join()
         phases = eng.timings()
         free, total = torch.cuda.mem_get_info()
         n_a, n, bits_a = index_sizes(eng)
         n_b = n - n_a
         passes_a = -(-bits_a // 10)
         per = {}
-        for e in prof.events():
+        events = [e for e in prof.events() if e.device_type == torch.autograd.DeviceType.CUDA]
+        split = any("SplitHistogramKernel" in e.name for e in events)
+        for e in events:
             if e.device_type != torch.autograd.DeviceType.CUDA:
                 continue
             if not any(k in e.name for k in KERNELS):
@@ -115,7 +141,7 @@
         rows = []
         for name, (ms, cnt) in sorted(per.items(), key=lambda x: -x[1][0]):
             ms_step, launches = ms / a.steps, cnt / a.steps
-            b = algorithmic_bytes(name, n, n_a, n_b, passes_a)
+            b = algorithmic_bytes(name, n, n_a, n_b, passes_a, split)
             rate = (b / (ms_step * 1e-3) / 1e12) if b and ms_step > 0 else None
             short = name.replace("(anonymous namespace)::", "").replace("void ", "")
             short = short.replace("unsigned ", "u").replace("rvn::", "").split("(")[0]
@@ -125,7 +151,7 @@
                          "tb_per_s": None if rate is None else round(rate, 3)})
         print(f"\nbare_count={setting}: {a.steps} steps, n={n} n_a={n_a} n_b={n_b} "
               f"(tier A: {bits_a} bits, {passes_a} passes); device memory in use after the "
-              f"steps {(total - free) / 2**30:.2f} GiB")
+              f"steps {(total - free) / 2**30:.2f} GiB, peak during them {peak[0] / 2**30:.2f} GiB")
         print(f"  phases (last step, ms): index_sort {phases.get('index_sort', 0):.2f}  "
               f"index_table {phases.get('index_table', 0):.2f}")
         print(f"  {'kernel':<58} {'ms/step':>8} {'launch':>6} {'GB':>7} {'TB/s':>6}")
@@ -135,7 +161,8 @@
                   f"{'' if r['tb_per_s'] is None else r['tb_per_s']:>6}")
         report["settings"][setting] = {
             "n": n, "n_a": n_a, "n_b": n_b, "phases_ms": phases, "kernels": rows,
-            "device_mem_used_gib": round((total - free) / 2**30, 3)}
+            "device_mem_used_gib": round((total - free) / 2**30, 3),
+            "device_mem_peak_gib": round(peak[0] / 2**30, 3)}
     if a.out:
         os.makedirs(a.out, exist_ok=True)
         with open(os.path.join(a.out, "index_build_split.json"), "w") as f:
diff --git a/raven_b200/csrc/engine.cuh b/raven_b200/csrc/engine.cuh
--- a/raven_b200/csrc/engine.cuh
+++ b/raven_b200/csrc/engine.cuh
@@ -87,8 +87,7 @@
   bool i_is32 = false;
   int i_shift = 0;
   uint64_t i_limit = ~0ULL;
-  DevBuf<uint32_t> t_cnt;
-  DevBuf<uint64_t> t_off, t_aval, t_aorg, t_b0, t_b1, t_b2, t_narrow;
+  DevBuf<uint64_t> t_b1, t_b2, t_narrow, t_split;
   const uint32_t* t_sorted_b = nullptr;
   uint64_t t_nb = 0;
   bool t_b_sorted = true;
@@ -234,6 +233,24 @@
                   uint64_t n, int begin_bit, int end_bit);
 void RadixPartitionKeys(Ctx& c, const uint32_t* src, uint32_t* dst, uint64_t n, int begin_bit,
                         int end_bit, uint32_t* bin_start);
+struct RadixSplit {
+  const uint32_t* keys = nullptr;
+  uint64_t n = 0;
+  uint32_t limit = 0;
+  uint64_t n_a = 0, n_b = 0;
+  int a_bits = 0, b_bits = 0;
+  int b_begin[2] = {-1, -1};
+  int a_sub = 1, b_sub = 1;
+  const uint32_t* span_le = nullptr;
+  const uint32_t* a_bases = nullptr;
+  const uint32_t* b_bases[2] = {nullptr, nullptr};
+};
+RadixSplit RadixSplitKeys(Ctx& c, const uint32_t* keys, uint64_t n, uint32_t limit, int a_bits,
+                          int b_bits, int b_begin0, int b_begin1);
+int RadixSortPairsAtMost(Ctx& c, const RadixSplit& s, const uint64_t* src_vals, uint32_t* keys_a,
+                         uint32_t* keys_b, uint64_t* vals_a, uint64_t* vals_b);
+int RadixSortKeysAbove(Ctx& c, const RadixSplit& s, int j, uint32_t* keys_a, uint32_t* keys_b);
+void RadixPartitionKeysAbove(Ctx& c, const RadixSplit& s, uint32_t* dst, uint32_t* bin_start);
 uint64_t* IndexHistogram(Ctx& c);
 uint32_t ThresholdFromHistogram(Ctx& c, const uint64_t* h_hist, uint64_t n_keys,
                                 double frequency, bool* needs_long_runs);
diff --git a/raven_b200/csrc/index.cu b/raven_b200/csrc/index.cu
--- a/raven_b200/csrc/index.cu
+++ b/raven_b200/csrc/index.cu
@@ -157,80 +157,6 @@
   if (i < n) out[i] = static_cast<uint32_t>(in[i]);
 }
 
-constexpr uint32_t kTierTile = 4096;
-
-__global__ void __launch_bounds__(kThreads)
-TierCountKernel(const uint32_t* __restrict__ val, uint64_t n, uint32_t limit,
-                uint32_t* __restrict__ tile_cnt) {
-  __shared__ uint32_t sm[34];
-  const uint64_t base = static_cast<uint64_t>(blockIdx.x) * kTierTile;
-  uint32_t mine = 0;
-#pragma unroll
-  for (uint32_t i = 0; i < kTierTile / kThreads; ++i) {
-    const uint64_t idx = base + i * kThreads + threadIdx.x;
-    mine += (idx < n && val[idx] <= limit) ? 1u : 0u;
-  }
-  uint32_t total;
-  BlockExclusiveSum<uint32_t, kThreads>(mine, sm, &total);
-  if (threadIdx.x == 0) tile_cnt[blockIdx.x] = total;
-}
-
-__global__ void __launch_bounds__(kThreads, 4)
-TierScatterKernel(const uint32_t* __restrict__ val, const uint64_t* __restrict__ org, uint64_t n,
-                  uint32_t limit, const uint64_t* __restrict__ tile_off_a,
-                  uint32_t* __restrict__ a_val, uint64_t* __restrict__ a_org,
-                  uint32_t* __restrict__ b_val) {
-  __shared__ uint32_t warp_a[kThreads / 32];
-  const uint32_t lane = threadIdx.x & 31, warp = threadIdx.x >> 5;
-  constexpr uint32_t kWarpSpan = kTierTile / (kThreads / 32);
-  const uint64_t tile_base = static_cast<uint64_t>(blockIdx.x) * kTierTile;
-  const uint64_t warp_base = tile_base + warp * kWarpSpan;
-  uint32_t v[kWarpSpan / 32];
-  uint32_t cnt = 0;
-#pragma unroll
-  for (uint32_t i = 0; i < kWarpSpan / 32; ++i) {
-    const uint64_t idx = warp_base + i * 32 + lane;
-    v[i] = idx < n ? val[idx] : 0xFFFFFFFFu;
-  }
-#pragma unroll
-  for (uint32_t i = 0; i < kWarpSpan / 32; ++i) {
-    const uint64_t idx = warp_base + i * 32 + lane;
-    cnt += __popc(__ballot_sync(0xFFFFFFFFu, idx < n && v[i] <= limit));
-  }
-  if (lane == 0) warp_a[warp] = cnt;
-  __syncthreads();
-  uint64_t a_at = tile_off_a[blockIdx.x];
-  for (uint32_t w = 0; w < warp; ++w) a_at += warp_a[w];
-  uint64_t b_at = warp_base - a_at;
-#pragma unroll
-  for (uint32_t h = 0; h < kWarpSpan / 32; h += 8) {
-    uint64_t o[8];
-#pragma unroll
-    for (uint32_t u = 0; u < 8; ++u) {
-      const uint64_t idx = warp_base + (h + u) * 32 + lane;
-      o[u] = (idx < n && v[h + u] <= limit) ? org[idx] : 0;
-    }
-#pragma unroll
-    for (uint32_t u = 0; u < 8; ++u) {
-      const uint32_t i = h + u;
-      const uint64_t idx = warp_base + i * 32 + lane;
-      const bool in = idx < n;
-      const bool is_a = in && v[i] <= limit;
-      const uint32_t ma = __ballot_sync(0xFFFFFFFFu, is_a);
-      const uint32_t mb = __ballot_sync(0xFFFFFFFFu, in && !is_a);
-      const uint32_t below = (1u << lane) - 1u;
-      if (is_a) {
-        const uint64_t d = a_at + __popc(ma & below);
-        a_val[d] = v[i];
-        a_org[d] = o[u];
-      } else if (in) {
-        b_val[b_at + __popc(mb & below)] = v[i];
-      }
-      a_at += __popc(ma);
-      b_at += __popc(mb);
-    }
-  }
-}
 
 __global__ void MaxU64Kernel(const uint64_t* __restrict__ v, uint64_t n,
                              unsigned long long* __restrict__ out) {
@@ -577,31 +503,28 @@
   TimerBegin(c, "index_sort");
   if (tiered) {
     const uint32_t* src32 = static_cast<const uint32_t*>(src_val.p);
-    const uint64_t tiles = (n + kTierTile - 1) / kTierTile;
-    uint32_t* tcnt = c.t_cnt.reserve(tiles + 1);
-    uint64_t* toff = c.t_off.reserve(tiles + 2);
-    TierCountKernel<<<static_cast<unsigned>(tiles), kThreads, 0, c.stream>>>(src32, n, limit32,
-                                                                          tcnt);
-    ExclusiveScanU32(c, tcnt, toff, tiles);
-    n_a = ReadU64(c, toff + tiles);
-    n_b = n - n_a;
-    uint32_t* a_val = reinterpret_cast<uint32_t*>(c.t_aval.reserve(n_a / 2 + 2));
-    uint64_t* a_org = c.t_aorg.reserve(n_a + 1);
-    uint32_t* b_src = reinterpret_cast<uint32_t*>(c.t_b0.reserve(n_b / 2 + 2));
-    TierScatterKernel<<<static_cast<unsigned>(tiles), kThreads, 0, c.stream>>>(
-        src32, src_org, n, limit32, toff, a_val, a_org, b_src);
-    RVN_LAUNCH_CHECK();
-    c.launches += 2;
     int bits_a = 1;
     while (bits_a < key_bits && (value_limit >> bits_a) != 0) ++bits_a;
+    int b_begin[2] = {-1, -1};
+    if (bare) {
+      b_begin[0] = key_bits - (key_bits > 2 * kBareBucketBits ? kBareBucketBits : 1);
+    } else {
+      b_begin[0] = 0;
+      if (key_bits > 2 * kGroupLowBits) b_begin[1] = kGroupLowBits;
+    }
+    const RadixSplit split =
+        RadixSplitKeys(c, src32, n, limit32, bits_a, key_bits, b_begin[0], b_begin[1]);
+    n_a = split.n_a;
+    n_b = split.n_b;
     c.i_val.reserve(n_a / 2 + 2);
     c.i_val_alt.reserve(n_a / 2 + 2);
     c.i_org.reserve(n_a + 1);
     c.i_org_alt.reserve(n_a + 1);
     if (n_a > 0) {
-      const int where = RadixSortPairs(c, a_val, reinterpret_cast<uint32_t*>(c.i_val.get()),
-                                       reinterpret_cast<uint32_t*>(c.i_val_alt.get()), a_org,
-                                       c.i_org.get(), c.i_org_alt.get(), n_a, 0, bits_a);
+      const int where = RadixSortPairsAtMost(c, split, src_org,
+                                             reinterpret_cast<uint32_t*>(c.i_val.get()),
+                                             reinterpret_cast<uint32_t*>(c.i_val_alt.get()),
+                                             c.i_org.get(), c.i_org_alt.get());
       if (where == 1) {
         c.i_val.swap(c.i_val_alt);
         c.i_org.swap(c.i_org_alt);
@@ -612,12 +535,11 @@
       c.t_b2.release();
       c.t_b_low = 0;
       c.t_b_sorted = false;
-      sorted_b = n_b > 0 ? b_src : nullptr;
-      if (n_b > 0 && key_bits > 2 * kBareBucketBits) {
+      if (n_b > 0) {
         uint32_t* starts = c.t_bstart.reserve(1u << kBareBucketBits);
-        RadixPartitionKeys(c, b_src, b1, n_b, key_bits - kBareBucketBits, key_bits, starts);
+        RadixPartitionKeysAbove(c, split, b1, starts);
         sorted_b = b1;
-        bstart = starts;
+        if (key_bits > 2 * kBareBucketBits) bstart = starts;
       }
     } else {
       uint32_t* b2 = reinterpret_cast<uint32_t*>(c.t_b2.reserve(n_b / 2 + 2));
@@ -627,8 +549,8 @@
                       : 0;
       c.t_b_sorted = c.t_b_low == 0;
       if (n_b > 0) {
-        const int where = RadixSortKeys(c, b_src, b1, b2, n_b, c.t_b_low, key_bits);
-        sorted_b = where < 0 ? b_src : (where == 0 ? b1 : b2);
+        const int where = RadixSortKeysAbove(c, split, c.t_b_low ? 1 : 0, b1, b2);
+        sorted_b = where == 0 ? b1 : b2;
       }
     }
     c.t_sorted_b = sorted_b;
@@ -779,14 +701,10 @@
           reinterpret_cast<const uint32_t*>(c.i_val.get()), c.i_n,
           reinterpret_cast<unsigned long long*>(counter), out);
       if (c.t_sorted_b && c.t_nb && !c.t_b_sorted) {
-        uint32_t* bufs[3] = {reinterpret_cast<uint32_t*>(c.t_b0.get()),
-                             reinterpret_cast<uint32_t*>(c.t_b1.get()),
-                             reinterpret_cast<uint32_t*>(c.t_b2.get())};
-        uint32_t* src = nullptr;
-        for (uint32_t* p : bufs) {
-          if (p == c.t_sorted_b) src = p;
-        }
-        uint32_t* other = src == bufs[0] ? bufs[1] : bufs[0];
+        uint32_t* src = const_cast<uint32_t*>(c.t_sorted_b);
+        const bool in_b1 = src == reinterpret_cast<uint32_t*>(c.t_b1.get());
+        uint32_t* other = in_b1 ? reinterpret_cast<uint32_t*>(c.t_b2.reserve(c.t_nb / 2 + 2))
+                                : reinterpret_cast<uint32_t*>(c.t_b1.get());
         const int where = RadixSortKeys(c, src, other, src, c.t_nb, 0,
                                         static_cast<int>(2 * c.prm.k));
         c.t_sorted_b = where == 0 ? other : src;
diff --git a/raven_b200/csrc/radix.cu b/raven_b200/csrc/radix.cu
--- a/raven_b200/csrc/radix.cu
+++ b/raven_b200/csrc/radix.cu
@@ -1,4 +1,6 @@
 #include <algorithm>
+#include <cstring>
+#include <type_traits>
 
 #include "engine.cuh"
 
@@ -33,6 +35,13 @@
   return static_cast<uint32_t>((key ^ flip) >> begin) & mask;
 }
 
+enum Keep : int { kKeepAll = 0, kKeepAtMost = 1, kKeepAbove = 2 };
+
+template <int KEEP, typename KeyT>
+__device__ __forceinline__ bool Kept(KeyT key, KeyT limit) {
+  return KEEP == kKeepAll || (KEEP == kKeepAtMost ? key <= limit : key > limit);
+}
+
 template <typename KeyT>
 __global__ void __launch_bounds__(kThreads)
 RadixHistogramKernel(const KeyT* __restrict__ keys, uint64_t n, PassPlan plan, KeyT flip,
@@ -56,6 +65,117 @@
   __syncthreads();
   for (int i = threadIdx.x; i < total; i += kThreads) {
     if (sh_hist[i]) atomicAdd(&hist[i], static_cast<unsigned long long>(sh_hist[i]));
+  }
+}
+
+constexpr int kSplitTile = kThreads * 32;
+constexpr int kSplitSpan = 1024;
+
+__global__ void __launch_bounds__(kThreads)
+SplitHistogramKernel(const uint32_t* __restrict__ keys, uint64_t n, uint32_t limit, PassPlan a,
+                     PassPlan b, unsigned long long* __restrict__ hist,
+                     unsigned long long* __restrict__ n_le, uint32_t* __restrict__ span_le) {
+  extern __shared__ uint32_t sh_hist[];
+  __shared__ uint32_t sh_le;
+  __shared__ uint32_t queue[kWarps][64];
+  const int total = (a.n_passes + b.n_passes) * kBins;
+  for (int i = threadIdx.x; i < total; i += kThreads) sh_hist[i] = 0;
+  if (threadIdx.x == 0) sh_le = 0;
+  __syncthreads();
+  const uint32_t lane = threadIdx.x & 31, warp = threadIdx.x >> 5;
+  const uint32_t lanemask_lt = (1u << lane) - 1u;
+  uint32_t* hb = sh_hist + a.n_passes * kBins;
+  uint32_t* q = queue[warp];
+  auto more_a = [&](uint32_t k) {
+#pragma unroll
+    for (int j = 1; j < kMaxPasses; ++j) {
+      if (j < a.n_passes) {
+        atomicAdd(&sh_hist[j * kBins + Digit<uint32_t>(k, 0u, a.begin[j], (1u << a.bits[j]) - 1u)],
+                  1u);
+      }
+    }
+  };
+  uint32_t queued = 0, le = 0;
+  const uint64_t n_spans = (n + kSplitSpan - 1) / kSplitSpan;
+  for (uint64_t span = static_cast<uint64_t>(blockIdx.x) * kWarps + warp; span < n_spans;
+       span += static_cast<uint64_t>(gridDim.x) * kWarps) {
+    const uint64_t base = span * kSplitSpan;
+    uint32_t sle = 0;
+    for (int s0 = 0; s0 < kSplitSpan / 32; s0 += 4) {
+      uint32_t k4[4];
+#pragma unroll
+      for (int u = 0; u < 4; ++u) {
+        const uint64_t i = base + (s0 + u) * 32 + lane;
+        k4[u] = i < n ? keys[i] : 0u;
+      }
+#pragma unroll
+      for (int u = 0; u < 4; ++u) {
+        const uint32_t k = k4[u];
+        const bool valid = base + (s0 + u) * 32 + lane < n;
+        const bool in_a = valid && k <= limit;
+        if (valid) {
+          if (in_a) {
+            atomicAdd(&sh_hist[Digit<uint32_t>(k, 0u, a.begin[0], (1u << a.bits[0]) - 1u)], 1u);
+          } else {
+            atomicAdd(&hb[Digit<uint32_t>(k, 0u, b.begin[0], (1u << b.bits[0]) - 1u)], 1u);
+#pragma unroll
+            for (int j = 1; j < kMaxPasses; ++j) {
+              if (j < b.n_passes) {
+                atomicAdd(
+                    &hb[j * kBins + Digit<uint32_t>(k, 0u, b.begin[j], (1u << b.bits[j]) - 1u)], 1u);
+              }
+            }
+          }
+        }
+        const uint32_t m = __ballot_sync(0xFFFFFFFFu, in_a);
+        sle += __popc(m);
+        if (a.n_passes > 1) {
+          if (in_a) q[queued + __popc(m & lanemask_lt)] = k;
+          queued += __popc(m);
+          __syncwarp();
+          if (queued >= 32) {
+            more_a(q[lane]);
+            const uint32_t rest = queued - 32 > lane ? q[32 + lane] : 0u;
+            __syncwarp();
+            if (queued - 32 > lane) q[lane] = rest;
+            queued -= 32;
+            __syncwarp();
+          }
+        }
+      }
+    }
+    if (lane == 0) span_le[span] = sle;
+    le += sle;
+  }
+  if (lane < queued) more_a(q[lane]);
+  if (lane == 0 && le) atomicAdd(&sh_le, le);
+  __syncthreads();
+  for (int i = threadIdx.x; i < total; i += kThreads) {
+    if (sh_hist[i]) atomicAdd(&hist[i], static_cast<unsigned long long>(sh_hist[i]));
+  }
+  if (threadIdx.x == 0 && sh_le) atomicAdd(n_le, static_cast<unsigned long long>(sh_le));
+}
+
+constexpr int kMaxSubTiles = 4;
+
+__global__ void SplitTileMaxKernel(const uint32_t* __restrict__ span_le, uint64_t n_tiles,
+                                   uint64_t n, uint32_t* __restrict__ most) {
+  constexpr int kSpans = kSplitTile / kSplitSpan;
+  const uint64_t t = static_cast<uint64_t>(blockIdx.x) * blockDim.x + threadIdx.x;
+  if (t >= n_tiles) return;
+  const uint64_t n_spans = (n + kSplitSpan - 1) / kSplitSpan;
+  uint32_t le = 0;
+#pragma unroll
+  for (int m = 1; m <= kMaxSubTiles; ++m) {
+    for (int j = 0; j < kSpans; ++j) {
+      const uint64_t sp = (t + m - 1) * kSpans + j;
+      if (sp < n_spans) le += span_le[sp];
+    }
+    if (t % m == 0) {
+      const uint64_t in = min(static_cast<uint64_t>(m) * kSplitTile, n - t * kSplitTile);
+      atomicMax(&most[m - 1], le);
+      atomicMax(&most[kMaxSubTiles + m - 1], static_cast<uint32_t>(in - le));
+    }
   }
 }
 
@@ -136,7 +256,14 @@
                : "memory");
 }
 
-template <typename KeyT, typename ValT, bool HAS_VAL>
+template <typename KeyT, bool HAS_VAL, int kTile>
+struct KeptRecords {
+  KeyT keys[kTile];
+  uint16_t at[HAS_VAL ? kTile : 1];
+  uint16_t by_slot[HAS_VAL ? kTile : 1];
+};
+
+template <typename KeyT, typename ValT, bool HAS_VAL, bool kFiltered = false>
 struct __align__(16) PassSmem {
   static constexpr int kTile = kThreads * Items<KeyT>::value;
   uint16_t warp_hist[kWarps][kBins];
@@ -144,22 +271,25 @@
   uint32_t bin_dst[kBins];
   uint32_t scan[34];
   uint32_t tile;
-  uint16_t slot_digit[HAS_VAL ? kTile : 2];
+  uint16_t slot_digit[HAS_VAL && !kFiltered ? kTile : 2];
   union {
     KeyT keys[kTile];
     ValT vals[HAS_VAL ? kTile : 1];
+    std::conditional_t<kFiltered, KeptRecords<KeyT, HAS_VAL, kTile>, char> kept;
   } stage;
 };
 
-template <typename KeyT, typename ValT, bool HAS_VAL>
+template <typename KeyT, typename ValT, bool HAS_VAL, int KEEP = kKeepAll>
 __global__ void __launch_bounds__(kThreads, 2)
 OnesweepPass(const KeyT* __restrict__ keys_in, KeyT* __restrict__ keys_out,
              const ValT* __restrict__ vals_in, ValT* __restrict__ vals_out, uint32_t n,
              KeyT flip, int begin_bit, int pass_bits, const uint32_t* __restrict__ bin_base,
              uint32_t* __restrict__ bin_next, uint32_t* __restrict__ status,
-             unsigned int* __restrict__ ticket) {
+             unsigned int* __restrict__ ticket, KeyT limit, int sub_tiles,
+             const uint32_t* __restrict__ span_le) {
   extern __shared__ __align__(16) unsigned char smem_raw[];
-  using Smem = PassSmem<KeyT, ValT, HAS_VAL>;
+  constexpr bool kFiltered = KEEP != kKeepAll;
+  using Smem = PassSmem<KeyT, ValT, HAS_VAL, kFiltered>;
   constexpr int kItems = Items<KeyT>::value;
   constexpr int kTile = kThreads * kItems;
   constexpr int kWarpTile = 32 * kItems;
@@ -176,25 +306,77 @@
   }
   __syncthreads();
   const uint32_t tile = sm.tile;
-  const uint64_t tile_base = static_cast<uint64_t>(tile) * kTile;
-  const uint32_t tile_count =
-      static_cast<uint32_t>(min(static_cast<uint64_t>(kTile), static_cast<uint64_t>(n) - tile_base));
+  const uint32_t tile_span = kFiltered ? kTile * static_cast<uint32_t>(sub_tiles) : kTile;
+  const uint64_t tile_base = static_cast<uint64_t>(tile) * tile_span;
+  const uint32_t tile_count = static_cast<uint32_t>(
+      min(static_cast<uint64_t>(tile_span), static_cast<uint64_t>(n) - tile_base));
 
   KeyT key[kItems];
-  const uint32_t warp_base = warp * kWarpTile;
-#pragma unroll
-  for (int i = 0; i < kItems; ++i) {
-    const uint32_t t = warp_base + i * 32 + lane;
-    key[i] = t < tile_count ? keys_in[tile_base + t] : static_cast<KeyT>(0);
-  }
+  uint32_t warp_base = warp * kWarpTile;
+  if constexpr (!kFiltered) {
+#pragma unroll
+    for (int i = 0; i < kItems; ++i) {
+      const uint32_t t = warp_base + i * 32 + lane;
+      key[i] = t < tile_count ? keys_in[tile_base + t] : static_cast<KeyT>(0);
+    }
+  }
+
+  uint32_t count = tile_count;
+  int items = kItems;
+  if constexpr (kFiltered) {
+    static_assert(kWarpTile == kSplitSpan, "a warp's input records are one span of the split");
+    const uint32_t n_spans = (tile_count + kWarpTile - 1) / kWarpTile;
+    if (threadIdx.x < n_spans) {
+      const uint32_t le = span_le[tile_base / kWarpTile + threadIdx.x];
+      const uint32_t len = min(static_cast<uint32_t>(kWarpTile), tile_count - threadIdx.x * kWarpTile);
+      sm.scan[threadIdx.x] = KEEP == kKeepAtMost ? le : len - le;
+    }
+    __syncthreads();
+    count = 0;
+    for (uint32_t sp = 0; sp < n_spans; ++sp) count += sm.scan[sp];
+    uint32_t at = 0, next = 0;
+    for (uint32_t chunk = 0; chunk < tile_span; chunk += kTile) {
+      const uint32_t first_span = chunk / kWarpTile;
+      for (uint32_t sp = next; sp < first_span + warp && sp < n_spans; ++sp) at += sm.scan[sp];
+      next = max(next, first_span + warp);
+      const uint32_t c_base = chunk + warp_base;
+#pragma unroll
+      for (int i = 0; i < kItems; ++i) {
+        const uint32_t t = c_base + i * 32 + lane;
+        key[i] = t < tile_count ? keys_in[tile_base + t] : static_cast<KeyT>(0);
+      }
+#pragma unroll
+      for (int i = 0; i < kItems; ++i) {
+        const uint32_t t = c_base + i * 32 + lane;
+        const bool keep = t < tile_count && Kept<KEEP>(key[i], limit);
+        const uint32_t m = __ballot_sync(0xFFFFFFFFu, keep);
+        if (keep) {
+          const uint32_t s = at + __popc(m & lanemask_lt);
+          sm.stage.kept.keys[s] = key[i];
+          if (HAS_VAL) sm.stage.kept.at[s] = static_cast<uint16_t>(t);
+        }
+        at += __popc(m);
+      }
+      next = max(next, first_span + warp + 1);
+    }
+    __syncthreads();
+    items = static_cast<int>((count + kThreads - 1) / kThreads);
+    warp_base = warp * static_cast<uint32_t>(items) * 32;
+#pragma unroll
+    for (int i = 0; i < kItems; ++i) {
+      const uint32_t t = warp_base + i * 32 + lane;
+      if (i < items && t < count) key[i] = sm.stage.kept.keys[t];
+    }
+  }
+  auto valid_item = [&](int i, uint32_t t) { return (!kFiltered || i < items) && t < count; };
 
   constexpr int kHalf = kItems / 2;
-  ValT early[HAS_VAL ? kHalf : 1];
-  if (HAS_VAL) {
+  ValT early[HAS_VAL && !kFiltered ? kHalf : 1];
+  if (HAS_VAL && !kFiltered) {
 #pragma unroll
     for (int i = 0; i < kHalf; ++i) {
       const uint32_t t = warp_base + i * 32 + lane;
-      early[i] = t < tile_count ? vals_in[tile_base + t] : ValT(0);
+      early[i] = t < count ? vals_in[tile_base + t] : ValT(0);
     }
   }
 
@@ -202,8 +384,9 @@
   uint16_t* my_hist = sm.warp_hist[warp];
 #pragma unroll
   for (int i = 0; i < kItems; ++i) {
+    if (kFiltered && i >= items) break;
     const uint32_t t = warp_base + i * 32 + lane;
-    const bool valid = t < tile_count;
+    const bool valid = t < count;
     const uint32_t d = valid ? Digit<KeyT>(key[i], flip, begin_bit, dmask) : 0u;
     uint32_t peers = __ballot_sync(0xFFFFFFFFu, valid);
 #pragma unroll
@@ -264,12 +447,36 @@
 #pragma unroll
   for (int i = 0; i < kItems; ++i) {
     const uint32_t t = warp_base + i * 32 + lane;
-    if (t < tile_count) {
+    if (valid_item(i, t)) {
       const uint32_t d = Digit<KeyT>(key[i], flip, begin_bit, dmask);
       const uint32_t slot = sm.bin_off[d] + sm.warp_hist[warp][d] + rank[i];
       rank[i] = static_cast<uint16_t>(slot);
-      if (HAS_VAL) sm.slot_digit[slot] = static_cast<uint16_t>(d);
-    }
+      if constexpr (kFiltered) {
+        if (HAS_VAL) sm.stage.kept.by_slot[slot] = sm.stage.kept.at[t];
+      } else {
+        if (HAS_VAL) sm.slot_digit[slot] = static_cast<uint16_t>(d);
+      }
+    }
+  }
+
+  if constexpr (kFiltered) {
+#pragma unroll
+    for (int i = 0; i < kItems; ++i) {
+      const uint32_t t = warp_base + i * 32 + lane;
+      if (valid_item(i, t)) sm.stage.keys[rank[i]] = key[i];
+    }
+    __syncthreads();
+#pragma unroll
+    for (int i = 0; i < kItems; ++i) {
+      const uint32_t s = i * kThreads + threadIdx.x;
+      if (s < count) {
+        const KeyT k = sm.stage.keys[s];
+        const uint32_t dst = sm.bin_dst[Digit<KeyT>(k, flip, begin_bit, dmask)] + s;
+        keys_out[dst] = k;
+        if (HAS_VAL) vals_out[dst] = vals_in[tile_base + sm.stage.kept.by_slot[s]];
+      }
+    }
+    return;
   }
 
   if (HAS_VAL) {
@@ -277,23 +484,23 @@
 #pragma unroll
     for (int i = 0; i < kHalf; ++i) {
       const uint32_t t = warp_base + (kHalf + i) * 32 + lane;
-      late[i] = t < tile_count ? vals_in[tile_base + t] : ValT(0);
+      late[i] = t < count ? vals_in[tile_base + t] : ValT(0);
     }
 #pragma unroll
     for (int i = 0; i < kHalf; ++i) {
       const uint32_t t = warp_base + i * 32 + lane;
-      if (t < tile_count) sm.stage.vals[rank[i]] = early[i];
+      if (t < count) sm.stage.vals[rank[i]] = early[i];
     }
 #pragma unroll
     for (int i = 0; i < kHalf; ++i) {
       const uint32_t t = warp_base + (kHalf + i) * 32 + lane;
-      if (t < tile_count) sm.stage.vals[rank[kHalf + i]] = late[i];
+      if (t < count) sm.stage.vals[rank[kHalf + i]] = late[i];
     }
     __syncthreads();
 #pragma unroll
     for (int i = 0; i < kItems; ++i) {
       const uint32_t s = i * kThreads + threadIdx.x;
-      if (s < tile_count) vals_out[sm.bin_dst[sm.slot_digit[s]] + s] = sm.stage.vals[s];
+      if (s < count) vals_out[sm.bin_dst[sm.slot_digit[s]] + s] = sm.stage.vals[s];
     }
     __syncthreads();
   }
@@ -301,13 +508,13 @@
 #pragma unroll
   for (int i = 0; i < kItems; ++i) {
     const uint32_t t = warp_base + i * 32 + lane;
-    if (t < tile_count) sm.stage.keys[rank[i]] = key[i];
+    if (t < count) sm.stage.keys[rank[i]] = key[i];
   }
   __syncthreads();
 #pragma unroll
   for (int i = 0; i < kItems; ++i) {
     const uint32_t s = i * kThreads + threadIdx.x;
-    if (s < tile_count) {
+    if (s < count) {
       const KeyT k = sm.stage.keys[s];
       keys_out[sm.bin_dst[Digit<KeyT>(k, flip, begin_bit, dmask)] + s] = k;
     }
@@ -323,11 +530,12 @@
   uint32_t keys[kThreads * Items<uint32_t>::value];
 };
 
+template <bool kFiltered = false>
 __global__ void __launch_bounds__(kThreads, 2)
 PartitionPass(const uint32_t* __restrict__ keys_in, uint32_t* __restrict__ keys_out, uint32_t n,
               int begin_bit, int pass_bits, const uint32_t* __restrict__ bin_base,
               uint32_t* __restrict__ bin_next, uint32_t* __restrict__ status,
-              unsigned int* __restrict__ ticket) {
+              unsigned int* __restrict__ ticket, uint32_t limit) {
   extern __shared__ __align__(16) unsigned char smem_raw[];
   PartitionSmem& sm = *reinterpret_cast<PartitionSmem*>(smem_raw);
   constexpr int kItems = Items<uint32_t>::value;
@@ -356,7 +564,7 @@
 #pragma unroll
   for (int i = 0; i < kItems; ++i) {
     const uint32_t t = warp_base + i * 32 + lane;
-    if (t < tile_count) {
+    if (t < tile_count && (!kFiltered || key[i] > limit)) {
       rank[i] = static_cast<uint16_t>(atomicAdd(&sm.bin_cnt[(key[i] >> begin_bit) & dmask], 1u));
     }
   }
@@ -392,13 +600,15 @@
 #pragma unroll
   for (int i = 0; i < kItems; ++i) {
     const uint32_t t = warp_base + i * 32 + lane;
-    if (t < tile_count) sm.keys[sm.bin_off[(key[i] >> begin_bit) & dmask] + rank[i]] = key[i];
+    if (t < tile_count && (!kFiltered || key[i] > limit)) {
+      sm.keys[sm.bin_off[(key[i] >> begin_bit) & dmask] + rank[i]] = key[i];
+    }
   }
   __syncthreads();
 #pragma unroll
   for (int i = 0; i < kItems; ++i) {
     const uint32_t s = i * kThreads + threadIdx.x;
-    if (s < tile_count) {
+    if (s < (kFiltered ? total : tile_count)) {
       const uint32_t k = sm.keys[s];
       keys_out[sm.bin_dst[(k >> begin_bit) & dmask] + s] = k;
     }
@@ -421,23 +631,33 @@
   return plan;
 }
 
-template <typename KeyT, typename ValT, bool HAS_VAL>
+template <typename KeyT, typename ValT, bool HAS_VAL, int KEEP = kKeepAll>
 int SortImpl(Ctx& c, const KeyT* src_keys, KeyT* keys_a, KeyT* keys_b, const ValT* src_vals,
              ValT* vals_a, ValT* vals_b, uint64_t n, int begin_bit, int end_bit,
-             bool descending) {
-  if (n >= 0xFFFFFFFFULL) throw LimitError("radix sort of 2^32 or more records");
+             bool descending, const RadixSplit* split = nullptr,
+             const uint32_t* split_bases = nullptr) {
+  constexpr bool kFiltered = KEEP != kKeepAll;
+  const uint64_t n_in = kFiltered ? split->n : n;
+  if (n_in >= 0xFFFFFFFFULL) throw LimitError("radix sort of 2^32 or more records");
   const PassPlan plan = MakePlan(begin_bit, end_bit);
+  if (kFiltered && plan.n_passes == 0) throw InvalidArgument("radix sort of a split: no key bits");
   if (plan.n_passes == 0 || n == 0) return -1;
   using Smem = PassSmem<KeyT, ValT, HAS_VAL>;
+  using FirstSmem = PassSmem<KeyT, ValT, HAS_VAL, kFiltered>;
   constexpr uint64_t kTile = Smem::kTile;
   const KeyT flip = descending ? static_cast<KeyT>(~static_cast<KeyT>(0)) : static_cast<KeyT>(0);
   const uint64_t portion = ((1ULL << 30) - 1) / kTile * kTile;
   const uint64_t n_portions = (n + portion - 1) / portion;
-  const uint64_t max_tiles = (std::min(n, portion) + kTile - 1) / kTile;
+  const int sub = kFiltered ? (KEEP == kKeepAtMost ? split->a_sub : split->b_sub) : 1;
+  const uint64_t in_tile = kTile * static_cast<uint64_t>(sub);
+  const uint64_t in_portion = ((1ULL << 30) - 1) / in_tile * in_tile;
+  const uint64_t in_portions = (n_in + in_portion - 1) / in_portion;
+  const uint64_t max_tiles = std::max((std::min(n_in, in_portion) + in_tile - 1) / in_tile,
+                                      (std::min(n, portion) + kTile - 1) / kTile);
   const size_t hist_bytes = sizeof(uint64_t) * plan.n_passes * kBins;
   const size_t base_bytes = sizeof(uint32_t) * plan.n_passes * kBins;
   const size_t ticket_bytes = sizeof(unsigned int) * kMaxPasses * 8;
-  if (plan.n_passes * n_portions > kMaxPasses * 8) throw LimitError("radix sort: too many launches");
+  if (plan.n_passes * in_portions > kMaxPasses * 8) throw LimitError("radix sort: too many launches");
   const size_t status_bytes = sizeof(uint32_t) * max_tiles * kBins;
   const size_t head = hist_bytes + 2 * base_bytes + ticket_bytes;
   uint8_t* scratch = c.sort_tmp.reserve(head + status_bytes + 256);
@@ -447,17 +667,28 @@
   auto* ticket = reinterpret_cast<unsigned int*>(scratch + hist_bytes + 2 * base_bytes);
   auto* status = reinterpret_cast<uint32_t*>(scratch + head);
   RVN_CUDA(cudaMemsetAsync(scratch, 0, head, c.stream));
-  const unsigned hgrid =
-      static_cast<unsigned>(std::min<uint64_t>((n + kThreads - 1) / kThreads, c.sms * 8));
-  RadixHistogramKernel<KeyT><<<hgrid, kThreads, sizeof(uint32_t) * plan.n_passes * kBins,
-                               c.stream>>>(src_keys, n, plan, flip, hist);
-  RadixScanBinsKernel<<<1, kBins, 0, c.stream>>>(hist, plan.n_passes, bases[0]);
-  RVN_LAUNCH_CHECK();
-  c.launches += 2;
+  if (kFiltered) {
+    RVN_CUDA(cudaMemcpyAsync(bases[0], split_bases, base_bytes, cudaMemcpyDeviceToDevice,
+                             c.stream));
+  } else {
+    const unsigned hgrid =
+        static_cast<unsigned>(std::min<uint64_t>((n + kThreads - 1) / kThreads, c.sms * 8));
+    RadixHistogramKernel<KeyT><<<hgrid, kThreads, sizeof(uint32_t) * plan.n_passes * kBins,
+                                 c.stream>>>(src_keys, n, plan, flip, hist);
+    RadixScanBinsKernel<<<1, kBins, 0, c.stream>>>(hist, plan.n_passes, bases[0]);
+    RVN_LAUNCH_CHECK();
+    c.launches += 2;
+  }
 
   auto kern = OnesweepPass<KeyT, ValT, HAS_VAL>;
+  auto first_kern = OnesweepPass<KeyT, ValT, HAS_VAL, KEEP>;
   RVN_CUDA(cudaFuncSetAttribute(kern, cudaFuncAttributeMaxDynamicSharedMemorySize,
                                 static_cast<int>(sizeof(Smem))));
+  if (kFiltered) {
+    RVN_CUDA(cudaFuncSetAttribute(first_kern, cudaFuncAttributeMaxDynamicSharedMemorySize,
+                                  static_cast<int>(sizeof(FirstSmem))));
+  }
+  const KeyT limit = kFiltered ? static_cast<KeyT>(split->limit) : static_cast<KeyT>(0);
   const KeyT* kin = src_keys;
   const ValT* vin = src_vals;
   int where = -1;
@@ -466,16 +697,21 @@
     const int to = where == 0 ? 1 : 0;
     KeyT* kout = to == 0 ? keys_a : keys_b;
     ValT* vout = to == 0 ? vals_a : vals_b;
+    const bool filtered = kFiltered && p == 0;
+    const uint64_t len = filtered ? n_in : n;
     int cur = 0;
-    for (uint64_t q = 0; q < n_portions; ++q) {
-      const uint64_t first = q * portion;
-      const uint64_t cnt = std::min(portion, n - first);
-      const uint64_t tiles = (cnt + kTile - 1) / kTile;
+    const uint64_t part = filtered ? in_portion : portion;
+    const uint64_t tile_len = filtered ? in_tile : kTile;
+    for (uint64_t q = 0; q < (filtered ? in_portions : n_portions); ++q) {
+      const uint64_t first = q * part;
+      const uint64_t cnt = std::min(part, len - first);
+      const uint64_t tiles = (cnt + tile_len - 1) / tile_len;
       RVN_CUDA(cudaMemsetAsync(status, 0, sizeof(uint32_t) * tiles * kBins, c.stream));
-      kern<<<static_cast<unsigned>(tiles), kThreads, sizeof(Smem), c.stream>>>(
+      (filtered ? first_kern : kern)<<<static_cast<unsigned>(tiles), kThreads,
+                                       filtered ? sizeof(FirstSmem) : sizeof(Smem), c.stream>>>(
           kin + first, kout, HAS_VAL ? vin + first : vin, vout, static_cast<uint32_t>(cnt), flip,
           plan.begin[p], plan.bits[p], bases[cur] + p * kBins, bases[cur ^ 1] + p * kBins, status,
-          ticket + launch);
+          ticket + launch, limit, sub, filtered ? split->span_le + first / kSplitSpan : nullptr);
       RVN_LAUNCH_CHECK();
       ++c.launches;
       ++launch;
@@ -488,41 +724,11 @@
   return where;
 }
 
-}
-
-int RadixSortPairs(Ctx& c, const uint32_t* src_keys, uint32_t* keys_a, uint32_t* keys_b,
-                   const uint64_t* src_vals, uint64_t* vals_a, uint64_t* vals_b, uint64_t n,
-                   int begin_bit, int end_bit, bool descending) {
-  return SortImpl<uint32_t, uint64_t, true>(c, src_keys, keys_a, keys_b, src_vals, vals_a, vals_b,
-                                            n, begin_bit, end_bit, descending);
-}
-int RadixSortPairs(Ctx& c, const uint64_t* src_keys, uint64_t* keys_a, uint64_t* keys_b,
-                   const uint64_t* src_vals, uint64_t* vals_a, uint64_t* vals_b, uint64_t n,
-                   int begin_bit, int end_bit, bool descending) {
-  return SortImpl<uint64_t, uint64_t, true>(c, src_keys, keys_a, keys_b, src_vals, vals_a, vals_b,
-                                            n, begin_bit, end_bit, descending);
-}
-int RadixSortPairs(Ctx& c, const uint32_t* src_keys, uint32_t* keys_a, uint32_t* keys_b,
-                   const uint32_t* src_vals, uint32_t* vals_a, uint32_t* vals_b, uint64_t n,
-                   int begin_bit, int end_bit, bool descending) {
-  return SortImpl<uint32_t, uint32_t, true>(c, src_keys, keys_a, keys_b, src_vals, vals_a, vals_b,
-                                            n, begin_bit, end_bit, descending);
-}
-int RadixSortPairs(Ctx& c, const uint64_t* src_keys, uint64_t* keys_a, uint64_t* keys_b,
-                   const uint32_t* src_vals, uint32_t* vals_a, uint32_t* vals_b, uint64_t n,
-                   int begin_bit, int end_bit, bool descending) {
-  return SortImpl<uint64_t, uint32_t, true>(c, src_keys, keys_a, keys_b, src_vals, vals_a, vals_b,
-                                            n, begin_bit, end_bit, descending);
-}
-int RadixSortKeys(Ctx& c, const uint32_t* src_keys, uint32_t* keys_a, uint32_t* keys_b, uint64_t n,
-                  int begin_bit, int end_bit) {
-  return SortImpl<uint32_t, uint32_t, false>(c, src_keys, keys_a, keys_b, nullptr, nullptr, nullptr,
-                                             n, begin_bit, end_bit, false);
-}
-
-void RadixPartitionKeys(Ctx& c, const uint32_t* src, uint32_t* dst, uint64_t n, int begin_bit,
-                        int end_bit, uint32_t* bin_start) {
-  if (n >= 0xFFFFFFFFULL) throw LimitError("radix partition of 2^32 or more records");
+void PartitionImpl(Ctx& c, const uint32_t* src, uint32_t* dst, uint64_t n, int begin_bit,
+                   int end_bit, uint32_t* bin_start, const RadixSplit* split,
+                   const uint32_t* split_bases) {
+  const uint64_t n_in = split ? split->n : n;
+  if (n_in >= 0xFFFFFFFFULL) throw LimitError("radix partition of 2^32 or more records");
   if (end_bit - begin_bit < 1 || end_bit - begin_bit > kRadixMaxBits) {
     throw InvalidArgument("radix partition: 1 to 10 key bits");
   }
@@ -532,8 +738,8 @@
   plan.bits[0] = end_bit - begin_bit;
   constexpr uint64_t kTile = kThreads * Items<uint32_t>::value;
   const uint64_t portion = ((1ULL << 30) - 1) / kTile * kTile;
-  const uint64_t n_portions = (n + portion - 1) / portion;
-  const uint64_t max_tiles = (std::min(n, portion) + kTile - 1) / kTile;
+  const uint64_t n_portions = (n_in + portion - 1) / portion;
+  const uint64_t max_tiles = (std::min(n_in, portion) + kTile - 1) / kTile;
   const size_t hist_bytes = sizeof(uint64_t) * kBins;
   const size_t base_bytes = sizeof(uint32_t) * kBins;
   const size_t ticket_bytes = sizeof(unsigned int) * kMaxPasses * 8;
@@ -551,25 +757,32 @@
     RVN_CUDA(cudaMemsetAsync(bin_start, 0, base_bytes, c.stream));
     return;
   }
-  const unsigned hgrid =
-      static_cast<unsigned>(std::min<uint64_t>((n + kThreads - 1) / kThreads, c.sms * 8));
-  RadixHistogramKernel<uint32_t><<<hgrid, kThreads, sizeof(uint32_t) * kBins, c.stream>>>(
-      src, n, plan, 0u, hist);
-  RadixScanBinsKernel<<<1, kBins, 0, c.stream>>>(hist, 1, bases[0]);
-  RVN_LAUNCH_CHECK();
-  c.launches += 2;
+  if (split) {
+    RVN_CUDA(cudaMemcpyAsync(bases[0], split_bases, base_bytes, cudaMemcpyDeviceToDevice,
+                             c.stream));
+  } else {
+    const unsigned hgrid =
+        static_cast<unsigned>(std::min<uint64_t>((n + kThreads - 1) / kThreads, c.sms * 8));
+    RadixHistogramKernel<uint32_t><<<hgrid, kThreads, sizeof(uint32_t) * kBins, c.stream>>>(
+        src, n, plan, 0u, hist);
+    RadixScanBinsKernel<<<1, kBins, 0, c.stream>>>(hist, 1, bases[0]);
+    RVN_LAUNCH_CHECK();
+    c.launches += 2;
+  }
   RVN_CUDA(cudaMemcpyAsync(bin_start, bases[0], base_bytes, cudaMemcpyDeviceToDevice, c.stream));
-  RVN_CUDA(cudaFuncSetAttribute(PartitionPass, cudaFuncAttributeMaxDynamicSharedMemorySize,
+  auto kern = split ? PartitionPass<true> : PartitionPass<false>;
+  RVN_CUDA(cudaFuncSetAttribute(kern, cudaFuncAttributeMaxDynamicSharedMemorySize,
                                 static_cast<int>(sizeof(PartitionSmem))));
+  const uint32_t limit = split ? split->limit : 0u;
   int cur = 0;
   for (uint64_t q = 0; q < n_portions; ++q) {
     const uint64_t first = q * portion;
-    const uint64_t cnt = std::min(portion, n - first);
+    const uint64_t cnt = std::min(portion, n_in - first);
     const uint64_t tiles = (cnt + kTile - 1) / kTile;
     RVN_CUDA(cudaMemsetAsync(status, 0, sizeof(uint32_t) * tiles * kBins, c.stream));
-    PartitionPass<<<static_cast<unsigned>(tiles), kThreads, sizeof(PartitionSmem), c.stream>>>(
+    kern<<<static_cast<unsigned>(tiles), kThreads, sizeof(PartitionSmem), c.stream>>>(
         src + first, dst, static_cast<uint32_t>(cnt), plan.begin[0], plan.bits[0], bases[cur],
-        bases[cur ^ 1], status, ticket + q);
+        bases[cur ^ 1], status, ticket + q, limit);
     RVN_LAUNCH_CHECK();
     ++c.launches;
     cur ^= 1;
@@ -577,3 +790,135 @@
 }
 
 }
+
+int RadixSortPairs(Ctx& c, const uint32_t* src_keys, uint32_t* keys_a, uint32_t* keys_b,
+                   const uint64_t* src_vals, uint64_t* vals_a, uint64_t* vals_b, uint64_t n,
+                   int begin_bit, int end_bit, bool descending) {
+  return SortImpl<uint32_t, uint64_t, true>(c, src_keys, keys_a, keys_b, src_vals, vals_a, vals_b,
+                                            n, begin_bit, end_bit, descending);
+}
+int RadixSortPairs(Ctx& c, const uint64_t* src_keys, uint64_t* keys_a, uint64_t* keys_b,
+                   const uint64_t* src_vals, uint64_t* vals_a, uint64_t* vals_b, uint64_t n,
+                   int begin_bit, int end_bit, bool descending) {
+  return SortImpl<uint64_t, uint64_t, true>(c, src_keys, keys_a, keys_b, src_vals, vals_a, vals_b,
+                                            n, begin_bit, end_bit, descending);
+}
+int RadixSortPairs(Ctx& c, const uint32_t* src_keys, uint32_t* keys_a, uint32_t* keys_b,
+                   const uint32_t* src_vals, uint32_t* vals_a, uint32_t* vals_b, uint64_t n,
+                   int begin_bit, int end_bit, bool descending) {
+  return SortImpl<uint32_t, uint32_t, true>(c, src_keys, keys_a, keys_b, src_vals, vals_a, vals_b,
+                                            n, begin_bit, end_bit, descending);
+}
+int RadixSortPairs(Ctx& c, const uint64_t* src_keys, uint64_t* keys_a, uint64_t* keys_b,
+                   const uint32_t* src_vals, uint32_t* vals_a, uint32_t* vals_b, uint64_t n,
+                   int begin_bit, int end_bit, bool descending) {
+  return SortImpl<uint64_t, uint32_t, true>(c, src_keys, keys_a, keys_b, src_vals, vals_a, vals_b,
+                                            n, begin_bit, end_bit, descending);
+}
+int RadixSortKeys(Ctx& c, const uint32_t* src_keys, uint32_t* keys_a, uint32_t* keys_b, uint64_t n,
+                  int begin_bit, int end_bit) {
+  return SortImpl<uint32_t, uint32_t, false>(c, src_keys, keys_a, keys_b, nullptr, nullptr, nullptr,
+                                             n, begin_bit, end_bit, false);
+}
+
+void RadixPartitionKeys(Ctx& c, const uint32_t* src, uint32_t* dst, uint64_t n, int begin_bit,
+                        int end_bit, uint32_t* bin_start) {
+  PartitionImpl(c, src, dst, n, begin_bit, end_bit, bin_start, nullptr, nullptr);
+}
+
+RadixSplit RadixSplitKeys(Ctx& c, const uint32_t* keys, uint64_t n, uint32_t limit, int a_bits,
+                          int b_bits, int b_begin0, int b_begin1) {
+  if (n >= 0xFFFFFFFFULL) throw LimitError("radix split of 2^32 or more records");
+  RadixSplit s;
+  s.keys = keys;
+  s.n = n;
+  s.limit = limit;
+  s.a_bits = a_bits;
+  s.b_bits = b_bits;
+  s.b_begin[0] = b_begin0;
+  s.b_begin[1] = b_begin1;
+  PassPlan plan{};
+  int first[3] = {0, 0, 0};
+  const int begins[3] = {0, b_begin0, b_begin1};
+  const int ends[3] = {a_bits, b_bits, b_bits};
+  for (int j = 0; j < 3; ++j) {
+    first[j] = plan.n_passes;
+    if (begins[j] < 0) continue;
+    const PassPlan pj = MakePlan(begins[j], ends[j]);
+    if (pj.n_passes == 0) throw InvalidArgument("radix split: no key bits");
+    if (plan.n_passes + pj.n_passes > kMaxPasses) throw InvalidArgument("radix split: too many passes");
+    for (int p = 0; p < pj.n_passes; ++p) {
+      plan.begin[plan.n_passes] = pj.begin[p];
+      plan.bits[plan.n_passes] = pj.bits[p];
+      ++plan.n_passes;
+    }
+  }
+  const int a_passes = first[1];
+  const size_t hist_words = static_cast<size_t>(kMaxPasses) * kBins;
+  const size_t count_words = 1 + kMaxSubTiles;
+  const uint64_t n_tiles = (n + kSplitTile - 1) / kSplitTile;
+  const size_t tile_words = (n + kSplitSpan - 1) / kSplitSpan / 2 + 1;
+  uint64_t* buf = c.t_split.reserve(hist_words + count_words + hist_words / 2 + tile_words);
+  auto* hist = reinterpret_cast<unsigned long long*>(buf);
+  auto* n_le = reinterpret_cast<unsigned long long*>(buf + hist_words);
+  auto* most = reinterpret_cast<uint32_t*>(buf + hist_words + 1);
+  auto* bases = reinterpret_cast<uint32_t*>(buf + hist_words + count_words);
+  auto* span_le = reinterpret_cast<uint32_t*>(buf + hist_words + count_words + hist_words / 2);
+  RVN_CUDA(cudaMemsetAsync(buf, 0, sizeof(uint64_t) * (hist_words + count_words), c.stream));
+  if (n > 0) {
+    const unsigned hgrid =
+        static_cast<unsigned>(std::min<uint64_t>((n + kThreads - 1) / kThreads, c.sms * 8));
+    PassPlan b = plan;
+    for (int p = a_passes; p < plan.n_passes; ++p) {
+      b.begin[p - a_passes] = plan.begin[p];
+      b.bits[p - a_passes] = plan.bits[p];
+    }
+    b.n_passes = plan.n_passes - a_passes;
+    PassPlan a = plan;
+    a.n_passes = a_passes;
+    SplitHistogramKernel<<<hgrid, kThreads, sizeof(uint32_t) * plan.n_passes * kBins, c.stream>>>(
+        keys, n, limit, a, b, hist, n_le, span_le);
+    RadixScanBinsKernel<<<1, kBins, 0, c.stream>>>(hist, plan.n_passes, bases);
+    SplitTileMaxKernel<<<static_cast<unsigned>((n_tiles + 255) / 256), 256, 0, c.stream>>>(
+        span_le, n_tiles, n, most);
+    RVN_LAUNCH_CHECK();
+    c.launches += 3;
+  }
+  uint64_t counts[count_words];
+  RVN_CUDA(cudaMemcpyAsync(counts, n_le, sizeof(counts), cudaMemcpyDeviceToHost, c.stream));
+  RVN_CUDA(cudaStreamSynchronize(c.stream));
+  s.n_a = counts[0];
+  s.span_le = span_le;
+  s.n_b = n - s.n_a;
+  uint32_t h_most[2 * kMaxSubTiles];
+  std::memcpy(h_most, counts + 1, sizeof(h_most));
+  for (int m = 2; m <= kMaxSubTiles; ++m) {
+    if (h_most[m - 1] <= static_cast<uint32_t>(kSplitTile)) s.a_sub = m;
+    if (h_most[kMaxSubTiles + m - 1] <= static_cast<uint32_t>(kSplitTile)) s.b_sub = m;
+  }
+  s.a_bases = bases;
+  s.b_bases[0] = b_begin0 < 0 ? nullptr : bases + static_cast<size_t>(first[1]) * kBins;
+  s.b_bases[1] = b_begin1 < 0 ? nullptr : bases + static_cast<size_t>(first[2]) * kBins;
+  return s;
+}
+
+int RadixSortPairsAtMost(Ctx& c, const RadixSplit& s, const uint64_t* src_vals, uint32_t* keys_a,
+                         uint32_t* keys_b, uint64_t* vals_a, uint64_t* vals_b) {
+  return SortImpl<uint32_t, uint64_t, true, kKeepAtMost>(c, s.keys, keys_a, keys_b, src_vals,
+                                                         vals_a, vals_b, s.n_a, 0, s.a_bits,
+                                                         false, &s, s.a_bases);
+}
+
+int RadixSortKeysAbove(Ctx& c, const RadixSplit& s, int j, uint32_t* keys_a, uint32_t* keys_b) {
+  if (!s.b_bases[j]) throw InvalidArgument("radix split: that sort was not histogrammed");
+  return SortImpl<uint32_t, uint32_t, false, kKeepAbove>(c, s.keys, keys_a, keys_b, nullptr,
+                                                         nullptr, nullptr, s.n_b, s.b_begin[j],
+                                                         s.b_bits, false, &s, s.b_bases[j]);
+}
+
+void RadixPartitionKeysAbove(Ctx& c, const RadixSplit& s, uint32_t* dst, uint32_t* bin_start) {
+  if (!s.b_bases[0]) throw InvalidArgument("radix split: the partition was not histogrammed");
+  PartitionImpl(c, s.keys, dst, s.n_b, s.b_begin[0], s.b_bits, bin_start, &s, s.b_bases[0]);
+}
+
+}
```
